# linnil1/KIR_graph

Hardware: AMD Instinct MI355X
Metric: typed 150 bp PE reads/s (pileup+EM) per GPU; achieved HBM GB/s vs roofline (higher is better)
Workload: dtype f64

## Files before the change

include/graphkir_hip.h:

```cpp
#ifndef GRAPHKIR_HIP_H
#define GRAPHKIR_HIP_H

#include <stddef.h>
#include <stdint.h>

#ifdef __cplusplus
extern "C" {
#endif

#define GK_ABI_VERSION 1

#define GK_OK 0
#define GK_ERR_NO_DEVICE (-1)
#define GK_ERR_HIP (-2)
#define GK_ERR_ARG (-3)
#define GK_ERR_ASSERT (-4)
#define GK_ERR_CAPACITY (-5)

#define GK_MAX_CIG 14
#define GK_MAX_MM 16
#define GK_MAX_INS 6
#define GK_MAX_EVENTS 22
#define GK_CIG_M 0
#define GK_CIG_I 1
// ... 23 lines not shown

#define GK_SPILLED 0xFF
#define GK_WIDE_CIG 128
#define GK_WIDE_MM 256
#define GK_WIDE_INS 120
#define GK_WIDE_EVENTS 384
typedef struct gk_mate_wide {
  uint32_t pos0;
  uint16_t flag;
  uint8_t ref;
  uint8_t nh;
  uint8_t nm;
  uint8_t rsv0;
  uint16_t n_cig;
  uint16_t n_mm;
  uint16_t n_ins;
  uint32_t cig[GK_WIDE_CIG];
  uint32_t mm[GK_WIDE_MM];
  uint32_t ins[GK_WIDE_INS];
  uint8_t rsv1[16];
} gk_mate_wide;

typedef struct gk_ctx gk_ctx;
typedef struct gk_index gk_index;
typedef struct gk_tab gk_tab;
typedef struct gk_lut gk_lut;
typedef uint64_t gk_dptr;

int gk_abi_version(void);
const char* gk_last_error(void);
int gk_device_count(int* n);
int gk_ctx_create(int device, gk_ctx** out);
int gk_ctx_create_priority(int device, int urgent, gk_ctx** out);
int gk_ctx_destroy(gk_ctx* ctx);
int gk_sync(gk_ctx* ctx);
int gk_device_memory(gk_ctx* ctx, int64_t* free_bytes, int64_t* total_bytes, int64_t* pool_cached_bytes);
int gk_malloc(gk_ctx* ctx, size_t bytes, gk_dptr* out);
int gk_free(gk_ctx* ctx, gk_dptr p);
int gk_memset(gk_ctx* ctx, gk_dptr p, int value, size_t bytes);
int gk_h2d(gk_ctx* ctx, gk_dptr dst, const void* src, size_t bytes);
int gk_d2h(gk_ctx* ctx, void* dst, gk_dptr src, size_t bytes);
int gk_d2d(gk_ctx* ctx, gk_dptr dst, gk_dptr src, size_t bytes);
int gk_timer_start(gk_ctx* ctx);
int gk_timer_stop_ms(gk_ctx* ctx, float* ms);
int gk_prof_enable(gk_ctx* ctx, int on);
int gk_prof_kernel_count(void);
const char* gk_prof_kernel_name(int id);
int gk_prof_collect(gk_ctx* ctx, int64_t* launches, double* total_ms);

int gk_index_create(gk_ctx* ctx, const uint64_t* key, int32_t n_var, const int32_t* gene_vbeg,
                    int32_t n_gene, gk_index** out);
int gk_index_destroy(gk_index* idx);

typedef struct gk_tab_info {
  int64_t n_pairs;
  int64_t n_valid;
  int64_t n_ids;
  int32_t n_novel;
  int32_t err_flags;
  gk_dptr d_pair_src;
  gk_dptr d_off;
  gk_dptr d_ids;
  gk_dptr d_pair_gene;
  gk_dptr d_pair_nh;
  gk_dptr d_novel_key;
} gk_tab_info;
int gk_tabulate(gk_ctx* ctx, gk_index* idx, gk_dptr d_mates, int64_t n_pairs, gk_tab** out);
int gk_tabulate_corrected(gk_ctx* ctx, gk_index* idx, gk_dptr d_mates, int64_t n_pairs, gk_dptr d_corr,
                          gk_dptr d_gene_pos0, gk_tab** out);
int gk_tabulate_spilled(gk_ctx* ctx, gk_index* idx, gk_dptr d_mates, int64_t n_pairs, gk_dptr d_corr,
                        gk_dptr d_gene_pos0, const gk_mate_wide* wide, const int64_t* spill_pair, int64_t n_spill,
                        gk_tab** out);
#define GK_COMPACT_STAGE_WORDS 4352
int gk_tabulate_compact(gk_ctx* ctx, gk_index* idx, gk_dptr d_compact, int64_t n_pairs, gk_dptr d_corr,
                        gk_dptr d_gene_pos0, const gk_mate_wide* wide, const int64_t* spill_pair, int64_t n_spill,
                        gk_tab** out);
int gk_tab_from_csr(gk_ctx* ctx, int32_t n_var_total, int64_t n_valid, const uint32_t* off, const uint32_t* ids,
                    const uint8_t* pair_gene, const uint8_t* pair_nh, gk_tab** out);
int gk_tab_get_info(gk_tab* tab, gk_tab_info* info);
int gk_tab_destroy(gk_tab* tab);

int gk_select_gene(gk_ctx* ctx, gk_tab* tab, int gene, int multiple, gk_dptr d_rows_out, int64_t* n_out);
int gk_select_nonempty(gk_ctx* ctx, gk_tab* tab, gk_dptr d_rows, int64_t n_rows, gk_dptr d_vflag,
                       gk_dptr d_rows_out, int64_t* n_out);

int gk_variant_count(gk_ctx* ctx, gk_tab* tab, gk_dptr d_rows, int64_t n_rows, gk_dptr d_vflag,
                     gk_dptr d_cnt);
int gk_variant_count_range(gk_ctx* ctx, gk_tab* tab, gk_dptr d_rows, int64_t n_rows, gk_dptr d_vflag,
                           gk_dptr d_cnt, int32_t vbeg, int32_t vend);
int gk_variant_correct(gk_ctx* ctx, gk_tab* tab, gk_dptr d_cnt, gk_dptr d_vflag);
int gk_variant_surviving(gk_ctx* ctx, gk_tab* tab, gk_dptr d_cnt, gk_dptr d_vflag, int64_t max_out,
                         int32_t* ord_out, uint32_t* pos_out, uint32_t* neg_out, int64_t* n_out);

int gk_variant_surviving_gene(gk_ctx* ctx, gk_tab* tab, gk_dptr d_cnt, gk_dptr d_vflag, int32_t gene, int32_t vbeg,
                              int32_t vend, int64_t max_out, int32_t* ord_out, uint32_t* pos_out, uint32_t* neg_out,
                              int64_t* n_out);
int gk_sample_prepare(gk_ctx* ctx, gk_tab* tab, int32_t multiple, gk_dptr d_vflag, gk_dptr d_cnt, gk_dptr d_rows,
                      int64_t* gene_off_out);
int gk_sample_prepare_all(gk_ctx* ctx, gk_tab* tab, int32_t multiple, gk_dptr d_vflag, gk_dptr d_cnt, gk_dptr d_rows,
                          int64_t* gene_off_out, int64_t max_out, int32_t* ord_out, uint32_t* pos_out, uint32_t* neg_out,
                          int64_t* n_out, uint64_t* novel_key_out);
int gk_sample_prepare_exon(gk_ctx* ctx, gk_tab* tab, int32_t multiple, gk_dptr d_vflag, gk_dptr d_cnt, gk_dptr d_rows,
                           int64_t* gene_off_out, int64_t max_out, int32_t* ord_out, uint32_t* pos_out, uint32_t* neg_out,
                           int64_t* n_out);
int gk_sample_prepare_exon_from(gk_ctx* ctx, gk_tab* tab, int32_t multiple, gk_dptr d_vflag, gk_dptr d_cnt, gk_dptr d_rows,
                                int64_t* gene_off_out, int64_t max_out, int32_t* ord_out, uint32_t* pos_out,
                                uint32_t* neg_out, int64_t* n_out, gk_dptr d_cnt_full);

int gk_compat(gk_ctx* ctx, gk_tab* tab, gk_dptr d_rows, int64_t n_rows, gk_dptr d_vflag,
              int32_t vbeg, int32_t vend, gk_dptr d_mask, int32_t words, int32_t n_allele, int32_t keep_empty,
              gk_dptr d_probs, gk_dptr d_miss, gk_dptr d_nvar);

int gk_novel_assign(gk_ctx* ctx, gk_dptr d_probs, int64_t n_rows, int32_t n_cols, const uint32_t* col_entries,
                    int32_t n_entries, gk_dptr d_code, uint16_t* code_out, uint32_t* count_out, int32_t* first_out);
int gk_novel_confusion(gk_ctx* ctx, gk_tab* tab, gk_dptr d_rows, int64_t n_rows, gk_dptr d_code, gk_dptr d_vflag,
                       int32_t vbeg, int32_t vend, gk_dptr d_carry, const int32_t* entry_col, const int32_t* entry_slot,
                       int32_t n_entries, int32_t n_slots, uint64_t* totals_out, int64_t max_out, int32_t* slot_out,
                       int32_t* ord_out, uint32_t* count_out, uint64_t* key_out, int64_t* n_out);

int gk_lut_create(gk_ctx* ctx, int32_t log2_capacity, gk_lut** out);
int gk_lut_destroy(gk_lut* lut);
int gk_lut_collect(gk_lut* lut, gk_dptr d_vals, int64_t n);
int gk_lut_pending(gk_lut* lut, int32_t* n_total, int32_t* n_known);
int gk_lut_export(gk_lut* lut, int32_t first, int32_t count, double* keys_out);
int gk_lut_define(gk_lut* lut, int32_t first, int32_t count, const double* log_vals);
int gk_lut_apply(gk_lut* lut, gk_dptr d_in, gk_dptr d_out, int64_t n);
typedef int (*gk_log10_fn)(const double* values, int64_t n, double* out);
int gk_lut_resolve(gk_lut* lut, gk_log10_fn log10_fn, int32_t* n_new, int32_t* n_known, int32_t* n_undefined);
int gk_lut_resolve_stored(gk_lut* lut, gk_log10_fn log10_fn, int32_t* n_new, int32_t* n_known, int32_t* n_undefined);
int gk_lut_known(gk_lut* lut, int32_t* n_known);
int gk_compat_log(gk_ctx* ctx, gk_tab* tab, gk_dptr d_rows, int64_t n_rows, gk_dptr d_vflag,
                  int32_t vbeg, int32_t vend, gk_dptr d_mask, int32_t words, int32_t n_allele, int32_t keep_empty,
                  gk_lut* lut, gk_dptr d_log);

int gk_maxsum(gk_ctx* ctx, gk_dptr d_L, int64_t n_rows, int64_t ld, const int32_t* ids, int32_t n_sets,
              int32_t c_prev, const int32_t* cols, int32_t n_cols, double* out);
int gk_fraction(gk_ctx* ctx, gk_dptr d_L, int64_t n_rows, int64_t ld, const int32_t* ids,
                int32_t n_sets, int32_t c, double* frac_out);
int gk_setmax(gk_ctx* ctx, gk_dptr d_L, int64_t n_rows, int64_t ld, const int32_t* ids, int32_t n_sets,
              int32_t c, gk_dptr d_P);

int gk_compat_log_miss(gk_ctx* ctx, gk_tab* tab, gk_dptr d_rows, int64_t n_rows, gk_dptr d_vflag,
                       int32_t vbeg, int32_t vend, gk_dptr d_mask, int32_t words, int32_t n_allele,
                       int32_t keep_empty, gk_lut* lut, gk_dptr d_log, gk_dptr d_miss8, int64_t ldm, gk_dptr d_flags);
int gk_miss_colsum(gk_ctx* ctx, gk_dptr d_miss8, int64_t ldm, int32_t n_cols, gk_dptr d_msum);
int gk_compat_log_miss_cols(gk_ctx* ctx, gk_tab* tab, gk_dptr d_rows, int64_t n_rows, gk_dptr d_vflag,
                            int32_t vbeg, int32_t vend, gk_dptr d_mask, int32_t words, int32_t n_allele,
                            int32_t keep_empty, gk_lut* lut, const int32_t* table_cols, int32_t n_table_cols,
                            gk_dptr d_log, gk_dptr d_miss8, int64_t ldm, gk_dptr d_flags);
int gk_compat_log_miss_narrow(gk_ctx* ctx, gk_tab* tab, gk_dptr d_rows, int64_t n_rows, gk_dptr d_vflag,
                              int32_t vbeg, int32_t vend, gk_dptr d_mask, int32_t words, int32_t n_allele,
                              int32_t keep_empty, gk_lut* lut, const int32_t* table_cols, int32_t n_table_cols,
                              gk_dptr d_log, gk_dptr d_miss8, int64_t ldm, gk_dptr d_flags, gk_dptr d_msum);
int gk_compat_patch(gk_ctx* ctx, gk_lut* lut, gk_dptr d_log, int64_t n_rows, int32_t n_allele, gk_dptr d_miss8,
                    int64_t ldm, gk_dptr d_flags);
int gk_compat_index(gk_ctx* ctx, gk_tab* tab, gk_dptr d_rows, int64_t n_rows, gk_dptr d_vflag, int32_t vbeg,
                    int32_t vend, gk_dptr d_mask, int32_t words, int32_t n_allele, int32_t keep_empty, gk_lut* lut,
                    gk_dptr d_lidx, gk_dptr d_miss8, int64_t ldm, gk_dptr d_flags);
int gk_expand_index(gk_ctx* ctx, gk_lut* lut, gk_dptr d_lidx, int64_t ldi, int64_t n_rows, int32_t n_allele, gk_dptr d_L,
                    int64_t ld);
int gk_bound_step(gk_ctx* ctx, gk_dptr d_miss8, int64_t ldm, int64_t n_rows, gk_dptr d_msum, const int32_t* ids,
                  int32_t n_sets, int32_t c_prev, const int32_t* cols, int32_t n_cols, const uint8_t* first,
                  int32_t top_n, int32_t cap, uint32_t* hdr_out, int32_t* idx_out, uint32_t* m_out);
int gk_setsum(gk_ctx* ctx, gk_dptr d_L, int64_t n_rows, int64_t ld, const int32_t* ids, int32_t n_sets, int32_t c,
              double* value_out, double* frac_out);

typedef int (*gk_argsort_fn)(const double* values, int64_t n, int64_t* order_out);
typedef struct gk_search gk_search;
int gk_search_run(gk_ctx* ctx, gk_dptr d_L, int64_t n_rows, int64_t ld, int32_t n_allele, gk_dptr d_miss8,
                  int64_t ldm, gk_dptr d_msum, const int32_t* cols, int32_t n_cols, int32_t n_steps, int32_t top_n,
                  gk_argsort_fn argsort, const double* colsum_in, gk_search** out);
typedef struct gk_gene_job {
  gk_dptr d_rows;
  int64_t n_rows;
  gk_dptr d_mask;
  gk_dptr d_L;
  gk_dptr d_miss8;
  int64_t ldm;
  gk_dptr d_msum;
  gk_dptr d_flags;
  gk_dptr d_lidx;
  int32_t vbeg, vend;
  int32_t words, n_allele;
  int32_t n_steps, top_n;
  int32_t bound_ok, passes;
  int32_t indexed, patches;
  int32_t table_of, n_step_cols;
  const int32_t* step_cols;
  const int32_t* step_cols_off;
  const int32_t* table_cols;
  int32_t n_table_cols;
} gk_gene_job;
int gk_sample_search(gk_ctx* ctx, gk_ctx** more_ctx, int32_t n_more, gk_tab* tab, gk_dptr d_vflag, gk_lut* lut,
                     gk_gene_job* jobs, int32_t n_jobs, gk_argsort_fn argsort, gk_log10_fn log10_fn, gk_search** out);
int gk_search_steps(gk_search* s, int32_t* n_steps);
int gk_search_info(gk_search* s, int32_t step, int32_t* n, int64_t* rows, int32_t* bounded);
int gk_search_copy(gk_search* s, int32_t step, double* value, double* sum_indv, int32_t* ids, double* frac);
int gk_search_export(gk_search* const* s, int32_t n, int64_t* totals, int64_t* meta, double* value, double* sum_indv,
                     double* frac, int32_t* ids);
int gk_search_colsum(gk_search* s, double* out);
int gk_search_log(gk_search* s, int64_t* out, int64_t capacity, int64_t* n_out);
int gk_search_destroy(gk_search* s);
int gk_site_verdict(const int64_t* pos, const int64_t* code, const uint8_t* negative, const int64_t* count, int64_t n,
                    int32_t cn, int32_t* homozygous);
int gk_site_verdict_tallies(const uint64_t* keys, int64_t n_keys, const int64_t* label_of_insert, int64_t n_insert,
                            const int32_t* ordinal, const uint32_t* positive, const uint32_t* negative, int64_t n,
                            int32_t cn, int32_t* homozygous);
int gk_site_verdict_genes(const uint64_t* keys, int64_t n_keys, const int64_t* label_of_insert, int64_t n_insert,
                          const int32_t* ordinal, const uint32_t* positive, const uint32_t* negative,
                          const int64_t* bounds, int32_t n_groups, const int32_t* cn, int32_t* homozygous);

int gk_em_sets(gk_ctx* ctx, gk_tab* tab, gk_dptr d_rows, int64_t n_rows, int32_t vbeg, int32_t vend,
               gk_dptr d_mask, int32_t words, gk_dptr d_sets_out );
int gk_em_distinct(gk_ctx* ctx, gk_dptr d_sets, int64_t n_rows, int32_t words, int32_t max_out,
                   uint32_t* sets_out, uint32_t* count_out, int32_t* n_out);
int gk_em_run(gk_ctx* ctx, const uint32_t* sets, const double* weight, int32_t n_sets, int32_t words,
              int32_t n_allele, int32_t iter_max, double diff_threshold, double* prob_out,
              int32_t* iters_out);
typedef struct gk_em_job {
  gk_dptr d_rows;
  int64_t n_rows;
  gk_dptr d_mask;
  int32_t vbeg, vend;
  int32_t words, n_allele;
  int32_t n_distinct, iterations;
} gk_em_job;
int gk_sample_em(gk_ctx* ctx, gk_tab* tab, gk_em_job* jobs, int32_t n_jobs, int32_t iter_max, double diff_threshold,
                 double* prob_out, int64_t* count_out);

typedef struct gk_boot_job {
  const uint32_t* sets;
  const uint32_t* count;
  int32_t n_sets;
  int32_t words;
  int32_t n_allele;
  uint32_t stream;
} gk_boot_job;
int gk_em_bootstrap(gk_ctx* ctx, const gk_boot_job* jobs, int32_t n_jobs, int32_t n_boot, uint64_t seed,
                    int32_t iter_max, double diff_threshold,
                    double* prob_out,
                    int32_t* iters_out,
                    uint32_t* counts_out);

int gk_boot_row_counts(gk_ctx* ctx, int64_t n_rows, int32_t n_boot, int32_t boot_first, uint64_t seed, uint32_t stream,
                       gk_dptr d_W, int64_t ldw);
int gk_weighted_sums(gk_ctx* ctx, gk_dptr d_V, int64_t ld, int64_t n_rows, int32_t n_sets, gk_dptr d_W, int64_t ldw,
                     int32_t n_boot, double* out);

int gk_call_fit(gk_ctx* ctx, gk_dptr d_miss8, int64_t ldm, int64_t n_rows, int32_t n_table_cols, const int32_t* cols,
                int32_t n_cols, uint64_t* hist_out , uint64_t* col_out , uint64_t* m_out ,
                gk_dptr d_min);
int gk_call_fit_extra(gk_ctx* ctx, gk_dptr d_miss8, int64_t ldm, int64_t n_rows, int32_t n_table_cols, gk_dptr d_min,
                      uint64_t* with_out );

int gk_call_coverage(gk_ctx* ctx, gk_tab* tab, gk_dptr d_mates, gk_dptr d_compact, gk_dptr d_rows, int64_t n_rows,
                     gk_dptr d_miss8, int64_t ldm, int32_t n_table_cols, const int32_t* cols, int32_t n_cols, int32_t gene,
                     int64_t gene_len, uint32_t* depth_out );

typedef struct gk_packer gk_packer;
int gk_packer_create(const char* const* gene_names, int32_t n_genes, const char* const* ins_strings,
                     int32_t n_ins, gk_packer** out);
int gk_packer_destroy(gk_packer* pk);
int gk_packer_feed(gk_packer* pk, const char* text, size_t n_bytes, int32_t final);
int gk_packer_counts(gk_packer* pk, int64_t* n_lines, int64_t* n_reads, int64_t* n_pairs, int64_t* n_strange,
                     int64_t* n_strings);
int gk_packer_error(gk_packer* pk, int32_t* kind, int64_t* line_index);
int gk_packer_set_output(gk_packer* pk, gk_mate* mates_out, int64_t capacity);
int gk_packer_records(gk_packer* pk, gk_mate* mates_out, int64_t* pair_lines_out);
int gk_packer_spilled(gk_packer* pk, int64_t* n_spilled_pairs);
int gk_packer_spill_records(gk_packer* pk, gk_mate_wide* wide_out, int64_t* pair_index_out);
const char* gk_packer_string(gk_packer* pk, int64_t i);

typedef struct gk_bam gk_bam;
int gk_bam_open(const char* path, int32_t name_sorted, gk_bam** out);
int gk_bam_close(gk_bam* bam);
int gk_bam_info(gk_bam* bam, int64_t* n_records, int64_t* header_bytes, int32_t* n_ref);
int gk_bam_header(gk_bam* bam, char* text_out, int64_t capacity);
int gk_bam_next(gk_bam* bam, char* text_out, int64_t capacity, int64_t* n_written);
int gk_bam_pack(gk_bam* bam, struct gk_packer* packer);
int gk_bam_write(const char* path, const char* sam_text, int64_t n_bytes, int32_t coordinate_sort);
int gk_bam_write_lines(const char* path, const char* header_text, int64_t n_header, const char* sam_text,
                       int64_t n_bytes, const int64_t* line_idx, int64_t n_lines, int32_t coordinate_sort);
int gk_json_write_reads(const char* path, const char* sam_text, int64_t n_bytes, const int64_t* pair_lines,
                        int64_t n_pairs, const int64_t* src, int64_t n_rows, const uint32_t* off,
                        const uint32_t* ids, const char* const* names, int64_t n_names,
                        const char* const* genes, int32_t n_genes, const uint8_t* gene_of, const uint8_t* nh);
int gk_bam_pileup(gk_bam* bam, const int64_t* gene_off, int32_t n_gene, uint32_t* counts_out);
int gk_bam_pileup_sites(const char* path, const int64_t* sites, int64_t n_sites, const uint64_t* name_keys,
                        const int32_t* key_group, int64_t n_keys, const int32_t* site_group, uint32_t* counts_out);
int gk_sam_name_keys(const char* sam_text, int64_t n_bytes, const int64_t* line_idx, int64_t n_lines, uint64_t* keys_out);
int gk_bam_write_lines_tagged(const char* path, const char* header_text, int64_t n_header, const char* rg_text,
                              int64_t n_rg, const char* sam_text, int64_t n_bytes, const int64_t* line_idx,
                              const int32_t* line_group, int64_t n_lines, const char* const* tags, int32_t n_tags,
                              int32_t coordinate_sort);

int gk_depth(gk_ctx* ctx, gk_tab* tab, gk_dptr d_mates, int32_t multiple, const int64_t* gene_off,
             int32_t n_gene, uint32_t* depth_out);
int gk_depth_compact(gk_ctx* ctx, gk_tab* tab, gk_dptr d_compact, int32_t multiple, const int64_t* gene_off,
                     int32_t n_gene, uint32_t* depth_out);

int gk_depth_write_tsv(const char* path, const char* const* genes, const int64_t* gene_off, int32_t n_genes,
                       const uint32_t* depth);

int gk_cn_fit(gk_ctx* ctx, const double* x, const double* density, int32_t bins, const double* bases,
              int32_t n_bases, const double* dev, int32_t n_cn, int32_t first_cn, double space,
              double* loglik_out);
int gk_cn_assign(gk_ctx* ctx, const double* x, int32_t bins, double base, const double* dev, int32_t n_cn,
                 int32_t first_cn, double space, int32_t* cn_of_bin_out);

typedef struct gk_comm gk_comm;
int gk_comm_unique_id(void* id_out, size_t capacity);
int gk_comm_create(gk_ctx* ctx, const void* id, size_t id_bytes, int32_t rank, int32_t world, gk_comm** out);
int gk_comm_destroy(gk_comm* comm);
int gk_allgather_f64(gk_comm* comm, const double* send, double* recv, int64_t n);
int gk_allreduce_max_f64(gk_comm* comm, double* inout, int64_t n);
int gk_comm_barrier(gk_comm* comm);

int gk_mates_compact(gk_ctx* ctx, gk_dptr d_mates, int64_t n_mates, gk_dptr* d_compact_out, int64_t* bytes_out);
int gk_mates_expand(gk_ctx* ctx, gk_dptr d_compact, int64_t n_mates, gk_dptr d_mates_out);
int gk_mates_compact_size(const gk_mate* mates, int64_t n_mates, int32_t n_threads, int64_t* n_words_out);
int gk_mates_compact_host(const gk_mate* mates, int64_t n_mates, int32_t n_threads, uint32_t* out, int64_t capacity_words);

int gk_host_alloc(size_t bytes, void** out);
int gk_host_free(void* p);
int gk_h2d_async(gk_ctx* ctx, gk_dptr dst, const void* src, size_t bytes);

#ifdef __cplusplus
}
#endif
#endif
```

kir_graph_amd/_lib.py:

```python
from __future__ import annotations

import ctypes as C
import threading
import os
from pathlib import Path

import numpy as np

LIB_NAME = "libgraphkir_hip.so"
_lib = None


class GkError(RuntimeError):
    """Error reported by the native library."""


class GkNoDevice(GkError):
    """No HIP device: the typing path cannot run (there is no CPU fallback)."""


_MM = np.dtype([("ref_off", "<u2"), ("base", "u1"), ("rsv", "u1")])
MATE_DTYPE = np.dtype([
    ("pos0", "<u4"), ("flag", "<u2"), ("ref", "u1"), ("nh", "u1"),
    ("nm", "u1"), ("n_cig", "u1"), ("n_mm", "u1"), ("n_ins", "u1"),
    ("cig", "<u2", (14,)), ("mm", _MM, (16,)), ("ins", "<u4", (6,)),
])
assert MATE_DTYPE.itemsize == 128

MATE_WIDE_DTYPE = np.dtype([
    ("pos0", "<u4"), ("flag", "<u2"), ("ref", "u1"), ("nh", "u1"), ("nm", "u1"), ("rsv0", "u1"),
    ("n_cig", "<u2"), ("n_mm", "<u2"), ("n_ins", "<u2"),
    ("cig", "<u4", (128,)), ("mm", "<u4", (256,)), ("ins", "<u4", (120,)), ("rsv1", "u1", (16,)),
])
assert MATE_WIDE_DTYPE.itemsize == 2048
SPILLED = 0xFF

CIG_M, CIG_I, CIG_D, CIG_S = 0, 1, 2, 4
NM_ABSENT = 255
MAX_CIG, MAX_MM, MAX_INS, MAX_EV = 14, 16, 6, 22
COMPACT_STAGE_WORDS = 4352


class GeneJob(C.Structure):
    _fields_ = [
        ("d_rows", C.c_uint64), ("n_rows", C.c_int64), ("d_mask", C.c_uint64), ("d_L", C.c_uint64),
        ("d_miss8", C.c_uint64), ("ldm", C.c_int64), ("d_msum", C.c_uint64), ("d_flags", C.c_uint64),
        ("d_lidx", C.c_uint64),
        ("vbeg", C.c_int32), ("vend", C.c_int32), ("words", C.c_int32), ("n_allele", C.c_int32),
        ("n_steps", C.c_int32), ("top_n", C.c_int32), ("bound_ok", C.c_int32), ("passes", C.c_int32),
        ("indexed", C.c_int32), ("patches", C.c_int32),
        ("table_of", C.c_int32), ("n_step_cols", C.c_int32), ("step_cols", C.c_void_p), ("step_cols_off", C.c_void_p),
        ("table_cols", C.c_void_p), ("n_table_cols", C.c_int32),
    ]


class EmJob(C.Structure):
    _fields_ = [
        ("d_rows", C.c_uint64), ("n_rows", C.c_int64), ("d_mask", C.c_uint64),
        ("vbeg", C.c_int32), ("vend", C.c_int32), ("words", C.c_int32), ("n_allele", C.c_int32),
        ("n_distinct", C.c_int32), ("iterations", C.c_int32),
    ]


class BootJob(C.Structure):
    _fields_ = [
        ("sets", C.c_void_p), ("count", C.c_void_p),
        ("n_sets", C.c_int32), ("words", C.c_int32), ("n_allele", C.c_int32), ("stream", C.c_uint32),
    ]


class TabInfo(C.Structure):
    _fields_ = [
        ("n_pairs", C.c_int64), ("n_valid", C.c_int64), ("n_ids", C.c_int64),
        ("n_novel", C.c_int32), ("err_flags", C.c_int32),
        ("d_pair_src", C.c_uint64), ("d_off", C.c_uint64), ("d_ids", C.c_uint64),
        ("d_pair_gene", C.c_uint64), ("d_pair_nh", C.c_uint64), ("d_novel_key", C.c_uint64),
    ]


def libPath() -> Path:
    return Path(__file__).resolve().parent / LIB_NAME


_SIGS = {
    "gk_abi_version": (C.c_int, []),
    "gk_last_error": (C.c_char_p, []),
    "gk_device_count": (C.c_int, [C.POINTER(C.c_int)]),
    "gk_ctx_create": (C.c_int, [C.c_int, C.POINTER(C.c_void_p)]),
    "gk_ctx_create_priority": (C.c_int, [C.c_int, C.c_int, C.POINTER(C.c_void_p)]),
    "gk_ctx_destroy": (C.c_int, [C.c_void_p]),
    "gk_sync": (C.c_int, [C.c_void_p]),
    "gk_device_memory": (C.c_int, [C.c_void_p, C.POINTER(C.c_int64), C.POINTER(C.c_int64), C.POINTER(C.c_int64)]),
    "gk_malloc": (C.c_int, [C.c_void_p, C.c_size_t, C.POINTER(C.c_uint64)]),
    "gk_free": (C.c_int, [C.c_void_p, C.c_uint64]),
    "gk_memset": (C.c_int, [C.c_void_p, C.c_uint64, C.c_int, C.c_size_t]),
    "gk_h2d": (C.c_int, [C.c_void_p, C.c_uint64, C.c_void_p, C.c_size_t]),
    "gk_d2h": (C.c_int, [C.c_void_p, C.c_void_p, C.c_uint64, C.c_size_t]),
    "gk_d2d": (C.c_int, [C.c_void_p, C.c_uint64, C.c_uint64, C.c_size_t]),
    "gk_timer_start": (C.c_int, [C.c_void_p]),
    "gk_timer_stop_ms": (C.c_int, [C.c_void_p, C.POINTER(C.c_float)]),
    "gk_prof_enable": (C.c_int, [C.c_void_p, C.c_int]),
    "gk_prof_kernel_count": (C.c_int, []),
    "gk_prof_kernel_name": (C.c_char_p, [C.c_int]),
    "gk_prof_collect": (C.c_int, [C.c_void_p, C.c_void_p, C.c_void_p]),
    "gk_index_create": (C.c_int, [C.c_void_p, C.c_void_p, C.c_int32, C.c_void_p, C.c_int32, C.POINTER(C.c_void_p)]),
    "gk_index_destroy": (C.c_int, [C.c_void_p]),
    "gk_tabulate": (C.c_int, [C.c_void_p, C.c_void_p, C.c_uint64, C.c_int64, C.POINTER(C.c_void_p)]),
    "gk_tabulate_spilled": (C.c_int, [C.c_void_p, C.c_void_p, C.c_uint64, C.c_int64, C.c_uint64, C.c_uint64,
                                     C.c_void_p, C.c_void_p, C.c_int64, C.POINTER(C.c_void_p)]),
    "gk_tabulate_corrected": (C.c_int, [C.c_void_p, C.c_void_p, C.c_uint64, C.c_int64, C.c_uint64, C.c_uint64,
                                        C.POINTER(C.c_void_p)]),
    "gk_tabulate_compact": (C.c_int, [C.c_void_p, C.c_void_p, C.c_uint64, C.c_int64, C.c_uint64, C.c_uint64,
                                     C.c_void_p, C.c_void_p, C.c_int64, C.POINTER(C.c_void_p)]),
    "gk_tab_from_csr": (C.c_int, [C.c_void_p, C.c_int32, C.c_int64, C.c_void_p, C.c_void_p, C.c_void_p, C.c_void_p,
                                  C.POINTER(C.c_void_p)]),
    "gk_tab_get_info": (C.c_int, [C.c_void_p, C.POINTER(TabInfo)]),
    "gk_tab_destroy": (C.c_int, [C.c_void_p]),
    "gk_select_gene": (C.c_int, [C.c_void_p, C.c_void_p, C.c_int, C.c_int, C.c_uint64, C.POINTER(C.c_int64)]),
    "gk_select_nonempty": (C.c_int, [C.c_void_p, C.c_void_p, C.c_uint64, C.c_int64, C.c_uint64, C.c_uint64,
                                     C.POINTER(C.c_int64)]),
    "gk_variant_count": (C.c_int, [C.c_void_p, C.c_void_p, C.c_uint64, C.c_int64, C.c_uint64, C.c_uint64]),
    "gk_variant_count_range": (C.c_int, [C.c_void_p, C.c_void_p, C.c_uint64, C.c_int64, C.c_uint64, C.c_uint64,
                                         C.c_int32, C.c_int32]),
    "gk_variant_surviving": (C.c_int, [C.c_void_p, C.c_void_p, C.c_uint64, C.c_uint64, C.c_int64, C.c_void_p,
                                       C.c_void_p, C.c_void_p, C.POINTER(C.c_int64)]),
    "gk_variant_surviving_gene": (C.c_int, [C.c_void_p, C.c_void_p, C.c_uint64, C.c_uint64, C.c_int32, C.c_int32, C.c_int32,
                                            C.c_int64, C.c_void_p, C.c_void_p, C.c_void_p, C.POINTER(C.c_int64)]),
    "gk_sample_prepare": (C.c_int, [C.c_void_p, C.c_void_p, C.c_int32, C.c_uint64, C.c_uint64, C.c_uint64, C.c_void_p]),
    "gk_sample_prepare_all": (C.c_int, [C.c_void_p, C.c_void_p, C.c_int32, C.c_uint64, C.c_uint64, C.c_uint64, C.c_void_p,
                                       C.c_int64, C.c_void_p, C.c_void_p, C.c_void_p, C.POINTER(C.c_int64), C.c_void_p]),
    "gk_variant_correct": (C.c_int, [C.c_void_p, C.c_void_p, C.c_uint64, C.c_uint64]),
    "gk_compat": (C.c_int, [C.c_void_p, C.c_void_p, C.c_uint64, C.c_int64, C.c_uint64, C.c_int32, C.c_int32,
                            C.c_uint64, C.c_int32, C.c_int32, C.c_int32, C.c_uint64, C.c_uint64, C.c_uint64]),
    "gk_lut_create": (C.c_int, [C.c_void_p, C.c_int32, C.POINTER(C.c_void_p)]),
    "gk_lut_destroy": (C.c_int, [C.c_void_p]),
    "gk_lut_collect": (C.c_int, [C.c_void_p, C.c_uint64, C.c_int64]),
    "gk_lut_pending": (C.c_int, [C.c_void_p, C.POINTER(C.c_int32), C.POINTER(C.c_int32)]),
    "gk_lut_export": (C.c_int, [C.c_void_p, C.c_int32, C.c_int32, C.c_void_p]),
    "gk_lut_define": (C.c_int, [C.c_void_p, C.c_int32, C.c_int32, C.c_void_p]),
    "gk_lut_apply": (C.c_int, [C.c_void_p, C.c_uint64, C.c_uint64, C.c_int64]),
    "gk_bam_open": (C.c_int, [C.c_char_p, C.c_int32, C.POINTER(C.c_void_p)]),
    "gk_bam_close": (C.c_int, [C.c_void_p]),
    "gk_bam_info": (C.c_int, [C.c_void_p, C.POINTER(C.c_int64), C.POINTER(C.c_int64), C.POINTER(C.c_int32)]),
    "gk_bam_header": (C.c_int, [C.c_void_p, C.c_char_p, C.c_int64]),
    "gk_bam_pileup": (C.c_int, [C.c_void_p, C.c_void_p, C.c_int32, C.c_void_p]),
    "gk_bam_pileup_sites": (C.c_int, [C.c_char_p, C.c_void_p, C.c_int64, C.c_void_p, C.c_void_p, C.c_int64, C.c_void_p,
                                      C.c_void_p]),
    "gk_sam_name_keys": (C.c_int, [C.c_char_p, C.c_int64, C.c_void_p, C.c_int64, C.c_void_p]),
    "gk_bam_write_lines_tagged": (C.c_int, [C.c_char_p, C.c_char_p, C.c_int64, C.c_char_p, C.c_int64, C.c_char_p,
                                            C.c_int64, C.c_void_p, C.c_void_p, C.c_int64, C.c_void_p, C.c_int32,
                                            C.c_int32]),
    "gk_novel_assign": (C.c_int, [C.c_void_p, C.c_uint64, C.c_int64, C.c_int32, C.c_void_p, C.c_int32, C.c_uint64,
                                  C.c_void_p, C.c_void_p, C.c_void_p]),
    "gk_novel_confusion": (C.c_int, [C.c_void_p, C.c_void_p, C.c_uint64, C.c_int64, C.c_uint64, C.c_uint64, C.c_int32,
                                     C.c_int32, C.c_uint64, C.c_void_p, C.c_void_p, C.c_int32, C.c_int32, C.c_void_p,
                                     C.c_int64, C.c_void_p, C.c_void_p, C.c_void_p, C.c_void_p, C.POINTER(C.c_int64)]),
    "gk_bam_write": (C.c_int, [C.c_char_p, C.c_char_p, C.c_int64, C.c_int32]),
    "gk_bam_write_lines": (C.c_int, [C.c_char_p, C.c_char_p, C.c_int64, C.c_char_p, C.c_int64, C.c_void_p, C.c_int64,
                                     C.c_int32]),
    "gk_json_write_reads": (C.c_int, [C.c_char_p, C.c_char_p, C.c_int64, C.c_void_p, C.c_int64, C.c_void_p, C.c_int64,
                                      C.c_void_p, C.c_void_p, C.c_void_p, C.c_int64, C.c_void_p, C.c_int32,
                                      C.c_void_p, C.c_void_p]),
    "gk_bam_pack": (C.c_int, [C.c_void_p, C.c_void_p]),
    "gk_bam_next": (C.c_int, [C.c_void_p, C.c_void_p, C.c_int64, C.POINTER(C.c_int64)]),
    "gk_compat_log": (C.c_int, [C.c_void_p, C.c_void_p, C.c_uint64, C.c_int64, C.c_uint64, C.c_int32, C.c_int32,
                                C.c_uint64, C.c_int32, C.c_int32, C.c_int32, C.c_void_p, C.c_uint64]),
    "gk_maxsum": (C.c_int, [C.c_void_p, C.c_uint64, C.c_int64, C.c_int64, C.c_void_p, C.c_int32, C.c_int32,
                            C.c_void_p, C.c_int32, C.c_void_p]),
    "gk_fraction": (C.c_int, [C.c_void_p, C.c_uint64, C.c_int64, C.c_int64, C.c_void_p, C.c_int32, C.c_int32,
                              C.c_void_p]),
    "gk_setmax": (C.c_int, [C.c_void_p, C.c_uint64, C.c_int64, C.c_int64, C.c_void_p, C.c_int32, C.c_int32,
                            C.c_uint64]),
    "gk_packer_create": (C.c_int, [C.c_void_p, C.c_int32, C.c_void_p, C.c_int32, C.POINTER(C.c_void_p)]),
    "gk_packer_destroy": (C.c_int, [C.c_void_p]),
    "gk_packer_feed": (C.c_int, [C.c_void_p, C.c_char_p, C.c_size_t, C.c_int32]),
    "gk_packer_counts": (C.c_int, [C.c_void_p, C.POINTER(C.c_int64), C.POINTER(C.c_int64), C.POINTER(C.c_int64),
                                   C.POINTER(C.c_int64), C.POINTER(C.c_int64)]),
    "gk_packer_error": (C.c_int, [C.c_void_p, C.POINTER(C.c_int32), C.POINTER(C.c_int64)]),
    "gk_packer_records": (C.c_int, [C.c_void_p, C.c_void_p, C.c_void_p]),
    "gk_packer_set_output": (C.c_int, [C.c_void_p, C.c_void_p, C.c_int64]),
    "gk_packer_spilled": (C.c_int, [C.c_void_p, C.POINTER(C.c_int64)]),
    "gk_packer_spill_records": (C.c_int, [C.c_void_p, C.c_void_p, C.c_void_p]),
    "gk_packer_string": (C.c_char_p, [C.c_void_p, C.c_int64]),
    "gk_depth": (C.c_int, [C.c_void_p, C.c_void_p, C.c_uint64, C.c_int32, C.c_void_p, C.c_int32, C.c_void_p]),
    "gk_depth_compact": (C.c_int, [C.c_void_p, C.c_void_p, C.c_uint64, C.c_int32, C.c_void_p, C.c_int32, C.c_void_p]),
    "gk_depth_write_tsv": (C.c_int, [C.c_char_p, C.c_void_p, C.c_void_p, C.c_int32, C.c_void_p]),
    "gk_cn_fit": (C.c_int, [C.c_void_p, C.c_void_p, C.c_void_p, C.c_int32, C.c_void_p, C.c_int32, C.c_void_p,
                            C.c_int32, C.c_int32, C.c_double, C.c_void_p]),
    "gk_cn_assign": (C.c_int, [C.c_void_p, C.c_void_p, C.c_int32, C.c_double, C.c_void_p, C.c_int32, C.c_int32,
                               C.c_double, C.c_void_p]),
    "gk_em_sets": (C.c_int, [C.c_void_p, C.c_void_p, C.c_uint64, C.c_int64, C.c_int32, C.c_int32, C.c_uint64,
                             C.c_int32, C.c_uint64]),
    "gk_em_distinct": (C.c_int, [C.c_void_p, C.c_uint64, C.c_int64, C.c_int32, C.c_int32, C.c_void_p, C.c_void_p,
                                 C.POINTER(C.c_int32)]),
    "gk_compat_log_miss_cols": (C.c_int, [C.c_void_p, C.c_void_p, C.c_uint64, C.c_int64, C.c_uint64, C.c_int32, C.c_int32,
                                          C.c_uint64, C.c_int32, C.c_int32, C.c_int32, C.c_void_p, C.c_void_p, C.c_int32,
                                          C.c_uint64, C.c_uint64, C.c_int64, C.c_uint64]),
    "gk_compat_log_miss_narrow": (C.c_int, [C.c_void_p, C.c_void_p, C.c_uint64, C.c_int64, C.c_uint64, C.c_int32, C.c_int32,
                                            C.c_uint64, C.c_int32, C.c_int32, C.c_int32, C.c_void_p, C.c_void_p, C.c_int32,
                                            C.c_uint64, C.c_uint64, C.c_int64, C.c_uint64, C.c_uint64]),
    "gk_compat_log_miss": (C.c_int, [C.c_void_p, C.c_void_p, C.c_uint64, C.c_int64, C.c_uint64, C.c_int32, C.c_int32,
                                     C.c_uint64, C.c_int32, C.c_int32, C.c_int32, C.c_void_p, C.c_uint64, C.c_uint64,
                                     C.c_int64, C.c_uint64]),
    "gk_miss_colsum": (C.c_int, [C.c_void_p, C.c_uint64, C.c_int64, C.c_int32, C.c_uint64]),
    "gk_compat_index": (C.c_int, [C.c_void_p, C.c_void_p, C.c_uint64, C.c_int64, C.c_uint64, C.c_int32, C.c_int32,
                                  C.c_uint64, C.c_int32, C.c_int32, C.c_int32, C.c_void_p, C.c_uint64, C.c_uint64,
                                  C.c_int64, C.c_uint64]),
    "gk_expand_index": (C.c_int, [C.c_void_p, C.c_void_p, C.c_uint64, C.c_int64, C.c_int64, C.c_int32, C.c_uint64,
                                  C.c_int64]),
    "gk_bound_step": (C.c_int, [C.c_void_p, C.c_uint64, C.c_int64, C.c_int64, C.c_uint64, C.c_void_p, C.c_int32,
                                C.c_int32, C.c_void_p, C.c_int32, C.c_void_p, C.c_int32, C.c_int32, C.c_void_p,
                                C.c_void_p, C.c_void_p]),
    "gk_setsum": (C.c_int, [C.c_void_p, C.c_uint64, C.c_int64, C.c_int64, C.c_void_p, C.c_int32, C.c_int32,
                            C.c_void_p, C.c_void_p]),
    "gk_search_run": (C.c_int, [C.c_void_p, C.c_uint64, C.c_int64, C.c_int64, C.c_int32, C.c_uint64, C.c_int64,
                                C.c_uint64, C.c_void_p, C.c_int32, C.c_int32, C.c_int32, C.c_void_p, C.c_void_p,
                                C.POINTER(C.c_void_p)]),
    "gk_sample_search": (C.c_int, [C.c_void_p, C.c_void_p, C.c_int32, C.c_void_p, C.c_uint64, C.c_void_p, C.c_void_p,
                                   C.c_int32, C.c_void_p, C.c_void_p, C.c_void_p]),
    "gk_lut_resolve": (C.c_int, [C.c_void_p, C.c_void_p, C.POINTER(C.c_int32), C.POINTER(C.c_int32),
                                 C.POINTER(C.c_int32)]),
    "gk_sample_prepare_exon": (C.c_int, [C.c_void_p, C.c_void_p, C.c_int32, C.c_uint64, C.c_uint64, C.c_uint64, C.c_void_p,
                                         C.c_int64, C.c_void_p, C.c_void_p, C.c_void_p, C.POINTER(C.c_int64)]),
    "gk_sample_prepare_exon_from": (C.c_int, [C.c_void_p, C.c_void_p, C.c_int32, C.c_uint64, C.c_uint64, C.c_uint64, C.c_void_p,
                                              C.c_int64, C.c_void_p, C.c_void_p, C.c_void_p, C.POINTER(C.c_int64), C.c_uint64]),
    "gk_sample_em": (C.c_int, [C.c_void_p, C.c_void_p, C.c_void_p, C.c_int32, C.c_int32, C.c_double, C.c_void_p, C.c_void_p]),
    "gk_mates_compact": (C.c_int, [C.c_void_p, C.c_uint64, C.c_int64, C.POINTER(C.c_uint64), C.POINTER(C.c_int64)]),
    "gk_mates_expand": (C.c_int, [C.c_void_p, C.c_uint64, C.c_int64, C.c_uint64]),
    "gk_mates_compact_size": (C.c_int, [C.c_void_p, C.c_int64, C.c_int32, C.POINTER(C.c_int64)]),
    "gk_mates_compact_host": (C.c_int, [C.c_void_p, C.c_int64, C.c_int32, C.c_void_p, C.c_int64]),
    "gk_compat_patch": (C.c_int, [C.c_void_p, C.c_void_p, C.c_uint64, C.c_int64, C.c_int32, C.c_uint64, C.c_int64, C.c_uint64]),
    "gk_lut_resolve_stored": (C.c_int, [C.c_void_p, C.c_void_p, C.POINTER(C.c_int32), C.POINTER(C.c_int32),
                                        C.POINTER(C.c_int32)]),
    "gk_lut_known": (C.c_int, [C.c_void_p, C.POINTER(C.c_int32)]),
    "gk_search_steps": (C.c_int, [C.c_void_p, C.POINTER(C.c_int32)]),
    "gk_search_info": (C.c_int, [C.c_void_p, C.c_int32, C.POINTER(C.c_int32), C.POINTER(C.c_int64),
                                 C.POINTER(C.c_int32)]),
    "gk_search_copy": (C.c_int, [C.c_void_p, C.c_int32, C.c_void_p, C.c_void_p, C.c_void_p, C.c_void_p]),
    "gk_search_export": (C.c_int, [C.c_void_p, C.c_int32, C.c_void_p, C.c_void_p, C.c_void_p, C.c_void_p, C.c_void_p, C.c_void_p]),
    "gk_search_colsum": (C.c_int, [C.c_void_p, C.c_void_p]),
    "gk_search_log": (C.c_int, [C.c_void_p, C.c_void_p, C.c_int64, C.POINTER(C.c_int64)]),
    "gk_search_destroy": (C.c_int, [C.c_void_p]),
    "gk_site_verdict_tallies": (C.c_int, [C.c_void_p, C.c_int64, C.c_void_p, C.c_int64, C.c_void_p, C.c_void_p, C.c_void_p,
                                         C.c_int64, C.c_int32, C.POINTER(C.c_int32)]),
    "gk_site_verdict_genes": (C.c_int, [C.c_void_p, C.c_int64, C.c_void_p, C.c_int64, C.c_void_p, C.c_void_p, C.c_void_p,
                                       C.c_void_p, C.c_int32, C.c_void_p, C.c_void_p]),
    "gk_site_verdict": (C.c_int, [C.c_void_p, C.c_void_p, C.c_void_p, C.c_void_p, C.c_int64, C.c_int32,
                                  C.POINTER(C.c_int32)]),
    "gk_comm_unique_id": (C.c_int, [C.c_void_p, C.c_size_t]),
    "gk_comm_create": (C.c_int, [C.c_void_p, C.c_void_p, C.c_size_t, C.c_int32, C.c_int32, C.POINTER(C.c_void_p)]),
    "gk_comm_destroy": (C.c_int, [C.c_void_p]),
    "gk_allgather_f64": (C.c_int, [C.c_void_p, C.c_void_p, C.c_void_p, C.c_int64]),
    "gk_allreduce_max_f64": (C.c_int, [C.c_void_p, C.c_void_p, C.c_int64]),
    "gk_comm_barrier": (C.c_int, [C.c_void_p]),
    "gk_host_alloc": (C.c_int, [C.c_size_t, C.POINTER(C.c_void_p)]),
    "gk_host_free": (C.c_int, [C.c_void_p]),
    "gk_h2d_async": (C.c_int, [C.c_void_p, C.c_uint64, C.c_void_p, C.c_size_t]),
    "gk_em_run": (C.c_int, [C.c_void_p, C.c_void_p, C.c_void_p, C.c_int32, C.c_int32, C.c_int32, C.c_int32,
                            C.c_double, C.c_void_p, C.POINTER(C.c_int32)]),
    "gk_em_bootstrap": (C.c_int, [C.c_void_p, C.c_void_p, C.c_int32, C.c_int32, C.c_uint64, C.c_int32, C.c_double,
                                  C.c_void_p, C.c_void_p, C.c_void_p]),
    "gk_boot_row_counts": (C.c_int, [C.c_void_p, C.c_int64, C.c_int32, C.c_int32, C.c_uint64, C.c_uint32, C.c_uint64,
                                     C.c_int64]),
    "gk_weighted_sums": (C.c_int, [C.c_void_p, C.c_uint64, C.c_int64, C.c_int64, C.c_int32, C.c_uint64, C.c_int64, C.c_int32,
                                   C.c_void_p]),
    "gk_call_fit": (C.c_int, [C.c_void_p, C.c_uint64, C.c_int64, C.c_int64, C.c_int32, C.c_void_p, C.c_int32, C.c_void_p,
                              C.c_void_p, C.c_void_p, C.c_uint64]),
    "gk_call_fit_extra": (C.c_int, [C.c_void_p, C.c_uint64, C.c_int64, C.c_int64, C.c_int32, C.c_uint64, C.c_void_p]),
    "gk_call_coverage": (C.c_int, [C.c_void_p, C.c_void_p, C.c_uint64, C.c_uint64, C.c_uint64, C.c_int64, C.c_uint64, C.c_int64,
                                   C.c_int32, C.c_void_p, C.c_int32, C.c_int32, C.c_int64, C.c_void_p]),
}

EXPORTED = sorted(_SIGS)

ARGSORT_FN = C.CFUNCTYPE(C.c_int, C.POINTER(C.c_double), C.c_int64, C.POINTER(C.c_int64))


def _numpy_argsort(values, n, order_out):
    try:
        v = np.ctypeslib.as_array(values, shape=(n,))
        np.ctypeslib.as_array(order_out, shape=(n,))[:] = np.argsort(v)
        return 0
    except Exception:
        return 1


NUMPY_ARGSORT = ARGSORT_FN(_numpy_argsort)

LOG10_FN = C.CFUNCTYPE(C.c_int, C.POINTER(C.c_double), C.c_int64, C.POINTER(C.c_double))


def _numpy_log10(values, n, out):
    try:
        v = np.ctypeslib.as_array(values, shape=(n,))
        with np.errstate(divide="ignore"):
            np.ctypeslib.as_array(out, shape=(n,))[:] = np.log10(v)
        return 0
    except Exception:
        return 1


NUMPY_LOG10 = LOG10_FN(_numpy_log10)


def lib():
    global _lib
    if _lib is None:
        path = libPath()
        if not path.exists():
            raise GkError(
                f"{path} is missing: build it with `python -c 'import __graft_entry__ as g; g.build()'` "
                "(hipcc --offload-arch=gfx950). The typing path has no CPU fallback.")
        handle = C.CDLL(str(path))
        for name, (res, args) in _SIGS.items():
            fn = getattr(handle, name)
            fn.restype, fn.argtypes = res, args
        if handle.gk_abi_version() != 1:
            raise GkError("libgraphkir_hip.so ABI version mismatch")
        _lib = handle
    return _lib


def check(rc: int) -> None:
    if rc == 0:
        return
    msg = lib().gk_last_error().decode(errors="replace")
    if rc == -1:
        raise GkNoDevice(msg)
    if rc == -4:
        raise AssertionError(msg)
    raise GkError(f"[{rc}] {msg}")


def _np_ptr(a: np.ndarray) -> C.c_void_p:
    return C.c_void_p(a.ctypes.data)


class DeviceBuffer:

    def __init__(self, dev: "Device", shape, dtype):
        self.dev = dev
        self.shape = tuple(int(s) for s in (shape if isinstance(shape, (tuple, list)) else (shape,)))
        self.dtype = np.dtype(dtype)
        self.nbytes = int(np.prod(self.shape, dtype=np.int64)) * self.dtype.itemsize
        p = C.c_uint64()
        check(lib().gk_malloc(dev.ctx, max(self.nbytes, 16), C.byref(p)))
        self.ptr = p.value

    @property
    def size(self) -> int:
        return int(np.prod(self.shape, dtype=np.int64))

    def upload(self, a: np.ndarray) -> "DeviceBuffer":
        a = np.ascontiguousarray(a, dtype=self.dtype)
        assert a.nbytes == self.nbytes, (a.shape, self.shape)
        if a.nbytes:
            check(lib().gk_h2d(self.dev.ctx, self.ptr, _np_ptr(a), a.nbytes))
# ... 175 lines not shown
```

kir_graph_amd/build.py:

```python
from __future__ import annotations

import os
import shutil
import subprocess
from pathlib import Path

PKG = Path(__file__).resolve().parent
ROOT = PKG.parent
SOURCES = ["gk_runtime.hip", "gk_scan.hip", "gk_tabulate.hip", "gk_typing.hip", "gk_lut.hip",
           "gk_search.hip", "gk_bound.hip", "gk_em.hip", "gk_cn.hip", "gk_depth.hip", "gk_sampack.cpp", "gk_bamread.cpp", "gk_textout.cpp",
           "gk_comm.cpp", "gk_hostsearch.cpp", "gk_novel.hip", "gk_boot.hip", "gk_callboot.hip", "gk_compat_narrow.hip",
           "gk_callfit.hip", "gk_callcov.hip"]


def hipcc() -> str:
    for cand in (os.environ.get("HIPCC"), shutil.which("hipcc"), "/opt/rocm/bin/hipcc"):
        if cand and Path(cand).exists():
            return cand
    raise RuntimeError("hipcc not found (set HIPCC)")


def outOfDate(lib: Path) -> bool:
    if not lib.exists():
        return True
    t = lib.stat().st_mtime
    deps = [PKG / "csrc" / s for s in SOURCES] + list((PKG / "csrc").glob("*.h")) + [ROOT / "include" / "graphkir_hip.h"]
    return any(d.stat().st_mtime > t for d in deps)


KERNEL_SOURCES = {
    "compat_kernel": ["gk_typing.hip", "gk_lut.h", "gk_common.h"],
    "patch_pending": ["gk_typing.hip", "gk_lut.h", "gk_common.h"],
    "compat_rows8": ["gk_compat_narrow.hip", "gk_lut.h", "gk_common.h"],
    "count_ids_genes": ["gk_typing.hip", "gk_common.h"],
    "flag_nonempty": ["gk_typing.hip", "gk_common.h"],
    "flag_pairs": ["gk_typing.hip", "gk_common.h"],
    "gather_pair_flags": ["gk_typing.hip", "gk_common.h"],
    "tab_count": ["gk_tabulate.hip", "gk_common.h"],
    "tab_emit": ["gk_tabulate.hip", "gk_common.h"],
    "tab_expand": ["gk_tabulate.hip", "gk_common.h"],
    "minsum_sad": ["gk_bound.hip", "gk_common.h"],
    "minsum_finish": ["gk_bound.hip", "gk_common.h"],
    "select_hist1": ["gk_bound.hip", "gk_common.h"],
    "select_hist2": ["gk_bound.hip", "gk_common.h"],
    "select_append": ["gk_bound.hip", "gk_common.h"],
    "setmin_u8": ["gk_bound.hip", "gk_common.h"],
    "fraction_chunks": ["gk_search.hip", "gk_common.h"],
    "setsum_leaves": ["gk_search.hip", "gk_common.h"],
    "fold_leaves": ["gk_search.hip", "gk_common.h"],
    "colsum_chunks": ["gk_search.hip", "gk_common.h"],
    "maxsum_chunks": ["gk_search.hip", "gk_common.h"],
    "combine_chunks": ["gk_search.hip", "gk_common.h"],
    "em_sets_groups": ["gk_em.hip", "gk_common.h"],
    "em_sets_hash": ["gk_em.hip", "gk_common.h"],
    "em_sets_verify": ["gk_em.hip", "gk_common.h"],
    "em_sets_emit": ["gk_em.hip", "gk_common.h"],
    "em_kernel_genes": ["gk_em.hip", "gk_squarem.h", "gk_common.h"],
    "novel_assign": ["gk_novel.hip", "gk_common.h"],
    "novel_confusion": ["gk_novel.hip", "gk_common.h"],
    "novel_compact": ["gk_novel.hip", "gk_common.h"],
    "boot_resample": ["gk_boot.hip", "gk_common.h"],
    "boot_em_batch": ["gk_boot.hip", "gk_squarem.h", "gk_common.h"],
    "callboot_draw": ["gk_callboot.hip", "gk_common.h"],
    "callboot_sums": ["gk_callboot.hip", "gk_common.h"],
    "callboot_fold": ["gk_callboot.hip", "gk_common.h"],
    "callfit_profile": ["gk_callfit.hip", "gk_common.h"],
    "callfit_extra": ["gk_callfit.hip", "gk_common.h"],
    "callcov_mark": ["gk_callcov.hip", "gk_common.h"],
    "callcov_mark_lds": ["gk_callcov.hip", "gk_common.h"],
    "callcov_finish": ["gk_callcov.hip", "gk_common.h"],
}


def sourceDigest(kernel: str | None = None) -> str:
    import hashlib
    h = hashlib.sha256()
    names = KERNEL_SOURCES.get(kernel or "")
    if names is None:
        files = sorted((PKG / "csrc").glob("*.hip")) + sorted((PKG / "csrc").glob("*.h"))
    else:
        files = [PKG / "csrc" / n for n in names]
    for f in files:
        h.update(f.name.encode())
        h.update(f.read_bytes())
    return h.hexdigest()[:16]


EXTRA_FLAGS: dict[str, list[str]] = {}


def buildNative(force: bool = False, verbose: bool = False) -> Path:
    lib = PKG / "libgraphkir_hip.so"
    if not force and not outOfDate(lib):
        return lib
    objdir = PKG / "csrc" / "build"
    objdir.mkdir(exist_ok=True)
    base = [hipcc(), "-O3", "--offload-arch=gfx950", "-std=c++17", "-fPIC", "-Wno-unused-value",
            "-Wno-unused-result", f"-I{ROOT / 'include'}", f"-I{PKG / 'csrc'}"]
    jobs = []
    for src in SOURCES:
        obj = objdir / (src.rsplit(".", 1)[0] + ".o")
        cmd = base + EXTRA_FLAGS.get(src, []) + ["-c", str(PKG / "csrc" / src), "-o", str(obj)]
        if verbose:
            print(" ".join(cmd))
        jobs.append((src, obj, subprocess.Popen(cmd, stdout=subprocess.PIPE, stderr=subprocess.PIPE, text=True)))
    failed = []
    for src, obj, proc in jobs:
        out, err = proc.communicate()
        if proc.returncode != 0:
            failed.append(f"{src}:\n{out}\n{err}")
    if failed:
        raise RuntimeError("hipcc failed:\n" + "\n".join(failed))
    link = [hipcc(), "--offload-arch=gfx950", "-shared", "-fPIC", "-o", str(lib)] + [str(o) for _, o, _ in jobs] + ["-lz", "-ldl"]
    if verbose:
        print(" ".join(link))
    res = subprocess.run(link, capture_output=True, text=True)
    if res.returncode != 0:
        raise RuntimeError(f"link failed:\n{res.stdout}\n{res.stderr}")
    return lib


if __name__ == "__main__":
    print(buildNative(force=True, verbose=True))
```

kir_graph_amd/csrc/gk_hostsearch.cpp:

```cpp
#include <algorithm>
#include <cmath>
#include <memory>
#include <numeric>
#include <string>
#include <unordered_map>
#include <unordered_set>
#include <chrono>
#include <sys/syscall.h>
#include <unistd.h>

#include "gk_calls.h"
#include "gk_lut.h"

namespace {

struct Step {
  int n = 0;
  int bounded = 0;
  std::vector<double> value, sum_indv, frac;
  std::vector<int32_t> ids;
  int64_t rows() const { return (int64_t)value.size(); }
};

inline double sum_small(const double* a, int n) {
// ... 24 lines not shown
    for (int a = 0; a < A && unique_cols; ++a) {
      if (seen[cols[a]]) unique_cols = false;
      seen[cols[a]] = 1;
    }
  }
  if (k <= 2 && n_allele <= 2048 && unique_cols) {
    std::vector<char> offered((size_t)n_allele, 0);
    for (int a = 0; a < A; ++a) offered[cols[a]] = 1;
    if (k == 1) {
      std::vector<int32_t> pos((size_t)n_allele, T);
      for (int t = T - 1; t >= 0; --t) pos[prev[t]] = t;
      for (int t = 0; t < T; ++t) {
        const int p = prev[t];
        if (pos[p] != t) continue;
        const bool free_pass = !offered[p];
        uint8_t* row = first.data() + (size_t)t * A;
        for (int a = 0; a < A; ++a) row[a] = (free_pass || pos[cols[a]] >= t) ? 1 : 0;
      }
      return;
    }
    std::vector<int32_t> pos((size_t)n_allele * n_allele, T);
    for (int t = T - 1; t >= 0; --t) {
      const int lo = std::min(prev[2 * t], prev[2 * t + 1]), hi = std::max(prev[2 * t], prev[2 * t + 1]);
      pos[(size_t)lo * n_allele + hi] = t;
      pos[(size_t)hi * n_allele + lo] = t;
    }
    for (int t = 0; t < T; ++t) {
      const int lo = std::min(prev[2 * t], prev[2 * t + 1]), hi = std::max(prev[2 * t], prev[2 * t + 1]);
      if (pos[(size_t)lo * n_allele + hi] != t) continue;
      const int32_t* by_hi = pos.data() + (size_t)hi * n_allele;
      const int32_t* by_lo = pos.data() + (size_t)lo * n_allele;
      const bool lo_off = offered[lo], hi_off = offered[hi];
      uint8_t* row = first.data() + (size_t)t * A;
      for (int a = 0; a < A; ++a) {
        const int c = cols[a];
        const bool dup = (by_hi[c] < t && lo_off) || (by_lo[c] < t && hi_off);
        row[a] = dup ? 0 : 1;
      }
    }
    return;
  }
  std::unordered_set<std::string> seen;
  seen.reserve((size_t)T * A * 2);
  std::vector<int32_t> key((size_t)k + 1);
  for (int t = 0; t < T; ++t)
    for (int a = 0; a < A; ++a) {
      std::copy(prev + (size_t)t * k, prev + (size_t)(t + 1) * k, key.begin());
      key[k] = cols[a];
      std::sort(key.begin(), key.end());
      std::string s((const char*)key.data(), key.size() * sizeof(int32_t));
      first[(size_t)t * A + a] = seen.insert(std::move(s)).second ? 1 : 0;
    }
}

struct Head {
  int c = 0;
  std::vector<int32_t> ids;
  std::vector<double> value;
  std::vector<double> sum_indv;
  std::vector<double> key2;
};

void fill_sums(Head& h, const double* colsum) {
  const int64_t n = (int64_t)h.value.size();
  h.sum_indv.resize((size_t)n * h.c);
  h.key2.resize((size_t)n);
  for (int64_t i = 0; i < n; ++i) {
    double* s = h.sum_indv.data() + (size_t)i * h.c;
    for (int j = 0; j < h.c; ++j) s[j] = colsum[h.ids[(size_t)i * h.c + j]];
    h.key2[i] = -sum_small(s, h.c);
  }
}

void contenders(const Head& h, int top_n, std::vector<int64_t>& contend) {
  const int64_t n = (int64_t)h.value.size();
  contend.clear();
  if (n <= top_n) {
    contend.resize((size_t)n);
    std::iota(contend.begin(), contend.end(), 0);
    return;
  }
  std::vector<int64_t> order((size_t)n);
  std::iota(order.begin(), order.end(), 0);
  std::stable_sort(order.begin(), order.end(), [&](int64_t a, int64_t b) {
    const double ka = -h.value[a], kb = -h.value[b];
    if (ka != kb) return ka < kb;
    return h.key2[a] < h.key2[b];
  });
  const int64_t b = order[top_n - 1];
  const double b1 = -h.value[b], b2 = h.key2[b];
  for (int64_t i = 0; i < n; ++i) {
    const double k1 = -h.value[i];
    if (k1 < b1 || (k1 == b1 && h.key2[i] <= b2)) contend.push_back(i);
  }
}

double unevenness(const double* f, int c) {
  const double mean = sum_small(f, c) / (double)c;
  double d[8];
  for (int j = 0; j < c; ++j) d[j] = std::fabs(f[j] - mean);
  return sum_small(d, c);
}

}

struct gk_search {
  int n_allele = 0;
  std::vector<int32_t> table_cols;
  int n_full = 0;
  std::vector<double> colsum;
  std::vector<Step> steps;
  std::vector<int64_t> log;
  int64_t distinct(const int32_t* ids, size_t n) const {
    std::vector<char> seen((size_t)n_allele, 0);
    int64_t d = 0;
    for (size_t i = 0; i < n; ++i)
      if (!seen[ids[i]]) { seen[ids[i]] = 1; ++d; }
    return d;
  }
  void note(int64_t kind, int64_t a, int64_t b, int64_t c, int64_t d, int64_t e, int64_t f) {
    const int64_t row[7] = {kind, a, b, c, d, e, f};
    log.insert(log.end(), row, row + 7);
  }
  void to_alleles(const int32_t* cols, int n_cols, int n_alleles) {
    for (Step& st : steps)
      for (int32_t& id : st.ids) id = cols[id];
    table_cols.assign(cols, cols + n_cols);
    n_full = n_alleles;
  }
};

extern "C" {

int gk_maxsum(gk_ctx* ctx, gk_dptr d_L, int64_t n_rows, int64_t ld, const int32_t* ids, int32_t n_sets, int32_t c_prev,
              const int32_t* cols, int32_t n_cols, double* out);
int gk_fraction(gk_ctx* ctx, gk_dptr d_L, int64_t n_rows, int64_t ld, const int32_t* ids, int32_t n_sets, int32_t c,
                double* frac_out);
int gk_compat_log_miss(gk_ctx* ctx, gk_tab* tab, gk_dptr d_rows, int64_t n_rows, gk_dptr d_vflag, int32_t vbeg,
                       int32_t vend, gk_dptr d_mask, int32_t words, int32_t n_allele, int32_t keep_empty, gk_lut* lut,
                       gk_dptr d_log, gk_dptr d_miss8, int64_t ldm, gk_dptr d_flags);
int gk_compat_log(gk_ctx* ctx, gk_tab* tab, gk_dptr d_rows, int64_t n_rows, gk_dptr d_vflag, int32_t vbeg,
                  int32_t vend, gk_dptr d_mask, int32_t words, int32_t n_allele, int32_t keep_empty, gk_lut* lut,
                  gk_dptr d_log);
__attribute__((weak)) int gk_compat_log_miss_cols(gk_ctx* ctx, gk_tab* tab, gk_dptr d_rows, int64_t n_rows, gk_dptr d_vflag,
                                                  int32_t vbeg, int32_t vend, gk_dptr d_mask, int32_t words, int32_t n_allele,
                                                  int32_t keep_empty, gk_lut* lut, const int32_t* table_cols,
                                                  int32_t n_table_cols, gk_dptr d_log, gk_dptr d_miss8, int64_t ldm,
                                                  gk_dptr d_flags);
__attribute__((weak)) int gk_compat_log_miss_narrow(gk_ctx* ctx, gk_tab* tab, gk_dptr d_rows, int64_t n_rows, gk_dptr d_vflag,
                                                    int32_t vbeg, int32_t vend, gk_dptr d_mask, int32_t words, int32_t n_allele,
                                                    int32_t keep_empty, gk_lut* lut, const int32_t* table_cols,
                                                    int32_t n_table_cols, gk_dptr d_log, gk_dptr d_miss8, int64_t ldm,
                                                    gk_dptr d_flags, gk_dptr d_msum);
int gk_miss_colsum(gk_ctx* ctx, gk_dptr d_miss8, int64_t ldm, int32_t n_cols, gk_dptr d_msum);
int gk_compat_patch(gk_ctx* ctx, gk_lut* lut, gk_dptr d_log, int64_t n_rows, int32_t n_allele, gk_dptr d_miss8, int64_t ldm,
                    gk_dptr d_flags);
int gk_compat_index(gk_ctx* ctx, gk_tab* tab, gk_dptr d_rows, int64_t n_rows, gk_dptr d_vflag, int32_t vbeg, int32_t vend,
                    gk_dptr d_mask, int32_t words, int32_t n_allele, int32_t keep_empty, gk_lut* lut, gk_dptr d_lidx,
                    gk_dptr d_miss8, int64_t ldm, gk_dptr d_flags);

}

namespace {

struct GeneSearch {
  gk_ctx* ctx = nullptr;
  GkTable table;
  gk_dptr d_L = 0;
  void* expanded = nullptr;
  gk_dptr d_miss8 = 0, d_msum = 0;
  int64_t n_rows = 0, ld = 0, ldm = 0;
  int n_allele = 0, n_steps = 0, T = 0, A = 0;
  std::vector<int32_t> cols;
  std::vector<std::vector<int32_t>> step_cols;
  gk_argsort_fn argsort = nullptr;
  bool bound = false, unique_cols = true;
  std::unique_ptr<gk_search> S;
  std::vector<uint8_t> first;
  int64_t N = 0;
  GkBoundCall bcall;
  GkSumCall scall;
  Head sel;
  Step st;
  bool bound_in_flight = false, sums_in_flight = false, step_done = false;

  int init(gk_ctx* c, const GkTable& tbl, gk_dptr L, int64_t rows, int64_t ld_, int32_t n_allele_, gk_dptr miss8, int64_t ldm_,
           gk_dptr msum, const int32_t* cols_, int32_t n_cols, int32_t n_steps_, int32_t top_n, gk_argsort_fn fn) {
    GK_REQUIRE(c && tbl.d && (L || tbl.indexed()) && cols_ && fn, "null pointer");
    table = tbl;
    GK_REQUIRE(rows > 0 && ld_ >= rows && n_allele_ > 0 && n_cols > 0 && n_steps_ >= 0 && n_steps_ <= 8 && top_n >= 1,
               "bad search arguments");
    for (int a = 0; a < n_cols; ++a) GK_REQUIRE(cols_[a] >= 0 && cols_[a] < n_allele_, "candidate allele out of range");
    ctx = c; d_L = L; n_rows = rows; ld = ld_; n_allele = n_allele_; d_miss8 = miss8; ldm = ldm_; d_msum = msum;
    cols.assign(cols_, cols_ + n_cols);
    n_steps = n_steps_; T = top_n; A = n_cols; argsort = fn;
    bound = d_miss8 != 0 && d_msum != 0;
    S.reset(new gk_search());
    S->n_allele = n_allele;
    S->colsum.resize((size_t)n_allele);
    std::vector<char> seen((size_t)n_allele, 0);
    for (int a = 0; a < A && unique_cols; ++a) { if (seen[cols[a]]) unique_cols = false; seen[cols[a]] = 1; }
    return GK_OK;
  }

  int use_step(int s) {
    if (step_cols.empty()) return GK_OK;
    const std::vector<int32_t>& c = step_cols[std::min<size_t>((size_t)s, step_cols.size() - 1)];
    GK_REQUIRE(!c.empty(), "a search step without candidate alleles");
    cols = c;
    A = (int)cols.size();
    unique_cols = true;
    std::vector<char> seen((size_t)n_allele, 0);
    for (int a = 0; a < A; ++a) {
      GK_REQUIRE(cols[a] >= 0 && cols[a] < n_allele, "candidate allele out of range");
      if (seen[cols[a]]) unique_cols = false;
      seen[cols[a]] = 1;
    }
    return GK_OK;
  }

  int colsum_enqueue() {
    std::vector<int32_t> every((size_t)n_allele);
    std::iota(every.begin(), every.end(), 0);
    int rc = gk_colsum_enqueue(ctx, table, n_rows, every.data(), n_allele, scall);
    if (rc) return rc;
    S->note(0, n_rows, 1, 0, n_allele, 0, 0);
    return GK_OK;
  }
  void colsum_collect() { gk_colsum_collect(ctx, scall, S->colsum.data()); }

  int first_step() {
    { const int r = use_step(0); if (r) return r; }
    const double* colsum = S->colsum.data();
    std::vector<double> score((size_t)A);
    for (int a = 0; a < A; ++a) score[a] = colsum[cols[a]];
    std::vector<int64_t> order((size_t)A);
    bool plain = true;
    for (int a = 0; a < A && plain; ++a) plain = score[a] == score[a];
    if (plain) {
      std::iota(order.begin(), order.end(), 0);
      std::sort(order.begin(), order.end(), [&](int64_t x, int64_t y) { return score[x] != score[y] ? score[x] < score[y] : x < y; });
      for (int a = 1; a < A && plain; ++a) plain = score[order[a - 1]] != score[order[a]];
    }
    if (!plain) GK_REQUIRE(argsort(score.data(), A, order.data()) == 0, "host argsort failed");
    Step s1;
    s1.n = 1;
    const int keep = std::min(T, A);
    for (int i = 0; i < keep; ++i) {
      const int64_t a = order[(size_t)A - 1 - i];
      GK_REQUIRE(a >= 0 && a < A, "host argsort returned an index out of range");
      s1.value.push_back(score[a]);
      s1.sum_indv.push_back(score[a]);
      s1.ids.push_back(cols[a]);
      s1.frac.push_back(1.0);
    }
    S->steps.push_back(std::move(s1));
    return GK_OK;
  }

  bool more() const { return (int)S->steps.size() < n_steps; }

  int step_begin() {
    { const int r = use_step((int)S->steps.size()); if (r) return r; }
    const Step& prev = S->steps.back();
    const int k = prev.n;
    const int Tp = (int)prev.rows();
    first_of_sets(prev.ids.data(), Tp, k, cols.data(), A, n_allele, first);
    N = 0;
    for (uint8_t f : first) N += f;
    st = Step();
    st.n = k + 1;
    step_done = bound_in_flight = sums_in_flight = false;
    if (bound && N > 0 && unique_cols) {
      const int cap = 4 * T + 4096;
      int rc = gk_bound_enqueue(ctx, d_miss8, ldm, n_rows, d_msum, prev.ids.data(), Tp, k, cols.data(), A, first.data(), T,
                                cap, bcall);
      if (rc) return rc;
      S->note(1, n_rows, Tp, A, k == 1 ? S->distinct(prev.ids.data(), prev.ids.size()) : Tp, 0, 0);
      bound_in_flight = true;
    }
    return GK_OK;
  }

  int after_bound() {
    if (!bound_in_flight) return GK_OK;
    bound_in_flight = false;
    const Step& prev = S->steps.back();
    const int k = prev.n, c = k + 1;
    const int cap = bcall.cap;
    uint32_t hdr[4];
    std::vector<int32_t> idx((size_t)cap);
    std::vector<uint32_t> mm((size_t)cap);
    gk_bound_collect(ctx, bcall, hdr, idx.data(), mm.data());
    const int64_t n_sel = hdr[2];
    if (n_sel <= 0 || n_sel > cap) return GK_OK;
    idx.resize((size_t)n_sel);
    std::sort(idx.begin(), idx.end());
    sel = Head();
    sel.c = c;
    sel.ids.resize((size_t)n_sel * c);
    for (int64_t i = 0; i < n_sel; ++i) {
      const int t = idx[i] / A, a = idx[i] % A;
      std::copy(prev.ids.begin() + (size_t)t * k, prev.ids.begin() + (size_t)(t + 1) * k, sel.ids.begin() + (size_t)i * c);
      sel.ids[(size_t)i * c + k] = cols[a];
    }
    int rc = gk_shares_enqueue(ctx, table, n_rows, sel.ids.data(), (int32_t)n_sel, c, true, scall);
// ... 270 lines not shown
  SearchClock clock("lock-step", (int)live.size());
  auto lap = [&](bool waited) { clock.lap(waited); };
  std::vector<uint32_t> flags((size_t)n_jobs, 0);
  std::vector<std::unique_ptr<GeneSearch>> gs((size_t)n_jobs);
  std::vector<char> sums_queued((size_t)n_jobs, 0);
  auto start_search = [&](int i, gk_dptr d_L, bool indexed) {
    gk_gene_job& j = jobs[i];
    std::vector<int32_t> cols((size_t)j.n_allele);
    std::iota(cols.begin(), cols.end(), 0);
    if (gs[i]) gs[i]->abandon();
    gs[i].reset(new GeneSearch());
    const GkTable tbl = indexed ? GkTable{j.d_lidx, j.ldm, lut->d_vals} : GkTable{d_L, j.n_rows, nullptr};
    int r = gs[i]->init(ctx_of[i], tbl, indexed ? 0 : d_L, j.n_rows, j.n_rows, j.n_allele, j.d_miss8, j.ldm, j.d_msum,
                        cols.data(), j.n_allele, j.n_steps, j.top_n, argsort);
    if (r == GK_OK) r = gs[i]->colsum_enqueue();
    sums_queued[i] = r == GK_OK;
    return r;
  };
  auto quit = [&](int code) {
    for (gk_ctx* c : cx) gk_fetch_cancel(c);
    for (auto& g : gs) if (g) g->abandon();
    return code;
  };
  std::vector<int> dirty(live);
  std::vector<uint32_t> sticky((size_t)n_jobs, 0);
  bool settled = false;
  for (int pass = 0; pass < 64 && !settled; ++pass) {
    int32_t known_at_launch = 0;
    rc = gk_lut_known(lut, &known_at_launch);
    if (rc) return quit(rc);
    for (int i : dirty) {
      gk_gene_job& j = jobs[i];
      gk_ctx* const gc = ctx_of[i];
      if (pass > 0 && j.d_L && j.d_miss8 && j.d_flags && (flags[i] & 12u) == 4u) {
        j.patches++;
        sticky[i] |= flags[i] & 1u;
        rc = gk_compat_patch(gc, lut, j.d_L, j.n_rows, j.n_allele, j.d_miss8, j.ldm, j.d_flags);
        if (rc == GK_OK) rc = gk_miss_colsum(gc, j.d_miss8, j.ldm, j.n_allele, j.d_msum);
        if (rc == GK_OK && gk_fetch_queue(gc, &flags[i], gk_ptr<void>(j.d_flags), sizeof(uint32_t)) != hipSuccess) rc = GK_ERR_HIP;
        if (rc == GK_OK) rc = start_search(i, j.d_L, false);
        if (rc) return quit(rc);
        continue;
      }
      j.passes++;
      sticky[i] = 0;
      if (j.d_lidx && !j.d_L) {
        rc = gk_compat_index(gc, tab, j.d_rows, j.n_rows, d_vflag, j.vbeg, j.vend, j.d_mask, j.words, j.n_allele, 0, lut,
                             j.d_lidx, j.d_miss8, j.ldm, j.d_flags);
        if (rc == GK_OK) rc = gk_miss_colsum(gc, j.d_miss8, j.ldm, j.n_allele, j.d_msum);
        if (rc == GK_OK && gk_fetch_queue(gc, &flags[i], gk_ptr<void>(j.d_flags), sizeof(uint32_t)) != hipSuccess) rc = GK_ERR_HIP;
      } else if (j.d_miss8) {
        rc = gk_compat_log_miss(gc, tab, j.d_rows, j.n_rows, d_vflag, j.vbeg, j.vend, j.d_mask, j.words, j.n_allele, 0, lut,
                                j.d_L, j.d_miss8, j.ldm, j.d_flags);
        if (rc == GK_OK) rc = gk_miss_colsum(gc, j.d_miss8, j.ldm, j.n_allele, j.d_msum);
        if (rc == GK_OK && gk_fetch_queue(gc, &flags[i], gk_ptr<void>(j.d_flags), sizeof(uint32_t)) != hipSuccess) rc = GK_ERR_HIP;
        if (rc == GK_OK) rc = start_search(i, j.d_L, false);
      } else {
        rc = gk_compat_log(gc, tab, j.d_rows, j.n_rows, d_vflag, j.vbeg, j.vend, j.d_mask, j.words, j.n_allele, 0, lut, j.d_L);
        if (rc == GK_OK) rc = start_search(i, j.d_L, false);
      }
      if (rc) return quit(rc);
    }
    lap(false); rc = wait_all(); lap(true);
    if (rc) return quit(rc);
    int32_t n_new = 0, n_known = 0, n_undefined = 0;
    rc = gk_lut_resolve(lut, log10_fn, &n_new, &n_known, &n_undefined);
    if (rc) return quit(rc);
    std::vector<int> again;
    bool unflagged = false;
    for (int i : dirty) {
      if (jobs[i].d_flags) { if (flags[i] & 4u) again.push_back(i); }
      else unflagged = true;
    }
    if (unflagged && (n_known > known_at_launch || n_undefined != 0))
      for (int i : dirty) if (!jobs[i].d_flags) again.push_back(i);
    std::sort(again.begin(), again.end());
    settled = again.empty();
    dirty.swap(again);
  }
  if (!settled) {
    gk_set_error("log10 value table did not settle");
    return quit(GK_ERR_ASSERT);
  }
  std::vector<void*> own_L((size_t)n_jobs, nullptr);
  auto fail = [&](int code) {
    for (gk_ctx* c : cx) gk_fetch_cancel(c);
    for (auto& g : gs) if (g) g->abandon();
    for (int i = 0; i < n_jobs; ++i) gk_pool_free(ctx_of[i], own_L[i]);
    return code;
  };
  for (int i : live) {
    gk_gene_job& j = jobs[i];
    j.indexed = (j.d_lidx && !j.d_L && !(flags[i] & 2u)) ? 1 : 0;
    if (j.d_lidx && !j.d_L && !j.indexed) {
      gk_ctx* const gc = ctx_of[i];
      if (gk_pool_malloc(gc, &own_L[i], (size_t)j.n_allele * (size_t)j.n_rows * sizeof(double)) != hipSuccess) {
        gk_set_error("out of device memory for the float64 table of a gene");
        return fail(GK_ERR_HIP);
      }
      rc = gk_compat_log_miss(gc, tab, j.d_rows, j.n_rows, d_vflag, j.vbeg, j.vend, j.d_mask, j.words, j.n_allele, 0, lut,
                              gk_addr(own_L[i]), j.d_miss8, j.ldm, j.d_flags);
      if (rc == GK_OK) rc = gk_miss_colsum(gc, j.d_miss8, j.ldm, j.n_allele, j.d_msum);
      if (rc == GK_OK && gk_fetch_queue(gc, &flags[i], gk_ptr<void>(j.d_flags), sizeof(uint32_t)) != hipSuccess) rc = GK_ERR_HIP;
      if (rc == GK_OK) rc = wait_stream(gc);
      if (rc) return fail(rc);
      j.passes++;
    }
  }
  bool late = false;
  for (int i : live) {
    gk_gene_job& j = jobs[i];
    j.bound_ok = (j.d_miss8 && ((flags[i] | sticky[i]) & 1u) == 0) ? 1 : 0;
    if (!sums_queued[i]) {
      rc = start_search(i, own_L[i] ? gk_addr(own_L[i]) : j.d_L, j.indexed != 0);
      if (rc) return fail(rc);
      late = true;
    }
    if (!j.bound_ok) gs[i]->bound = false;
  }
  if (late) {
    lap(false); rc = wait_all(); lap(true);
    if (rc) return fail(rc);
  }
  for (int i : live) {
    gs[i]->colsum_collect();
    rc = gs[i]->first_step();
    if (rc) return fail(rc);
  }
  for (;;) {
    std::vector<int> todo;
    for (int i : live) if (gs[i]->more()) todo.push_back(i);
    if (todo.empty()) break;
    for (int i : todo) { rc = gs[i]->step_begin(); if (rc) return fail(rc); }
    lap(false); rc = wait_all(); lap(true);
    if (rc) return fail(rc);
    for (int i : todo) { rc = gs[i]->after_bound(); if (rc) return fail(rc); }
    lap(false); rc = wait_all(); lap(true);
    if (rc) return fail(rc);
    for (int i : todo) { rc = gs[i]->after_sums(); if (rc) return fail(rc); }
    for (int i : todo) {
      if (!gs[i]->step_done) { rc = gs[i]->exact_step(); if (rc) return fail(rc); }
      gs[i]->step_end();
    }
  }
  for (int i : live) {
    gs[i]->finish();
    out[i] = gs[i]->S.release();
  }
  for (int i = 0; i < n_jobs; ++i) gk_pool_free(ctx_of[i], own_L[i]);
  lap(false);
  return GK_OK;
}

int sample_search_pipelined(gk_ctx* ctx, gk_tab* tab, gk_dptr d_vflag, gk_lut* lut, gk_gene_job* jobs, int32_t n_jobs,
                            const std::vector<int>& live, gk_argsort_fn argsort, gk_log10_fn log10_fn, gk_search** out) {
  SearchClock clock("pipelined", (int)live.size());
  std::vector<uint32_t> flags((size_t)n_jobs, 0);
  std::vector<std::unique_ptr<GeneSearch>> gs((size_t)n_jobs);
  enum { kTable, kBound, kSums, kOneSet };
  struct Item { int gene, stage; uint64_t mark; };
  std::deque<Item> queue;
  struct OneSetBatch { GkSumCall call; std::vector<int> deps; int k = 0; std::vector<int32_t> ids; };
  std::vector<std::unique_ptr<OneSetBatch>> batches;
  auto fail = [&](int code) {
    gk_fetch_cancel(ctx);
    for (auto& g : gs) if (g) g->abandon();
    for (auto& b : batches) if (b) gk_release(ctx, b->call.temps);
    return code;
  };
  auto push = [&](int gene, int stage) {
    uint64_t m = 0;
    const int r = set_mark(ctx, &m);
    if (r == GK_OK) queue.push_back({gene, stage, m});
    return r;
  };
  std::vector<uint32_t> sticky((size_t)n_jobs, 0);
  auto n_cols_of = [&](int i) { return jobs[i].n_table_cols > 0 ? jobs[i].n_table_cols : jobs[i].n_allele; };
  auto col_of = [&](int owner, int32_t a, int32_t* col) -> int {
    const gk_gene_job& o = jobs[owner];
    if (a < 0 || a >= o.n_allele) { gk_set_error("candidate allele out of range"); return GK_ERR_ARG; }
    if (o.n_table_cols <= 0) { *col = a; return GK_OK; }
    const int32_t* const end = o.table_cols + o.n_table_cols;
    const int32_t* const at = std::lower_bound(o.table_cols, end, a);
    if (at == end || *at != a) {
      gk_set_error("candidate allele %d is not among the columns of its table", (int)a);
      return GK_ERR_ARG;
    }
    *col = (int32_t)(at - o.table_cols);
    return GK_OK;
  };
  auto write_table = [&](int i, bool patch) -> int {
    gk_gene_job& j = jobs[i];
    const int nc = n_cols_of(i);
    int rc;
    bool summed = false;
    if (patch) {
      j.patches++;
      sticky[i] |= flags[i] & 1u;
      rc = gk_compat_patch(ctx, lut, j.d_L, j.n_rows, nc, j.d_miss8, j.ldm, j.d_flags);
    } else {
      j.passes++;
      sticky[i] = 0;
      static const bool wide_compat = gk_test_hook("wide_compat");
      if (j.n_table_cols > 0 && j.n_table_cols <= 8 && gk_compat_log_miss_narrow && !wide_compat) {
        rc = gk_compat_log_miss_narrow(ctx, tab, j.d_rows, j.n_rows, d_vflag, j.vbeg, j.vend, j.d_mask, j.words, j.n_allele, 0,
                                       lut, j.table_cols, j.n_table_cols, j.d_L, j.d_miss8, j.ldm, j.d_flags, j.d_msum);
        summed = true;
      } else if (j.n_table_cols > 0)
        rc = gk_compat_log_miss_cols(ctx, tab, j.d_rows, j.n_rows, d_vflag, j.vbeg, j.vend, j.d_mask, j.words, j.n_allele, 0,
                                     lut, j.table_cols, j.n_table_cols, j.d_L, j.d_miss8, j.ldm, j.d_flags);
      else
        rc = gk_compat_log_miss(ctx, tab, j.d_rows, j.n_rows, d_vflag, j.vbeg, j.vend, j.d_mask, j.words, j.n_allele, 0, lut,
                                j.d_L, j.d_miss8, j.ldm, j.d_flags);
    }
    if (rc == GK_OK && !summed) rc = gk_miss_colsum(ctx, j.d_miss8, j.ldm, nc, j.d_msum);
    if (rc == GK_OK && gk_fetch_queue(ctx, &flags[i], gk_ptr<void>(j.d_flags), sizeof(uint32_t)) != hipSuccess) rc = GK_ERR_HIP;
    if (rc) return rc;
    std::vector<int32_t> cols((size_t)nc);
    std::iota(cols.begin(), cols.end(), 0);
    if (gs[i]) gs[i]->abandon();
    gs[i].reset(new GeneSearch());
    rc = gs[i]->init(ctx, GkTable{j.d_L, j.n_rows, nullptr}, j.d_L, j.n_rows, j.n_rows, nc, j.d_miss8, j.ldm, j.d_msum,
                     cols.data(), nc, j.n_steps, j.top_n, argsort);
    if (rc == GK_OK) rc = gs[i]->colsum_enqueue();
    if (rc == GK_OK) rc = push(i, kTable);
    return rc;
  };
  std::vector<std::vector<int>> dependents((size_t)n_jobs);
  for (int i : live)
    if (jobs[i].table_of >= 0) dependents[(size_t)jobs[i].table_of].push_back(i);
  int rc = GK_OK;
  for (int i : live) {
    if (jobs[i].table_of >= 0) continue;
    rc = write_table(i, false);
    if (rc) return fail(rc);
  }

  auto advance = [&](int i, bool at_step_start) -> int {
    GeneSearch& g = *gs[i];
    for (;;) {
      if (at_step_start) {
        if (!g.more()) return GK_OK;
        const int r = g.step_begin();
        if (r) return r;
        if (g.bound_in_flight) return push(i, kBound);
      }
      if (!g.step_done) {
        const int r = g.exact_step();
        if (r) return r;
      }
      g.step_end();
      at_step_start = true;
    }
  };
  while (!queue.empty()) {
    const Item it = queue.front();
    queue.pop_front();
    clock.lap(false);
    rc = wait_mark(ctx, it.mark);
    clock.lap(true);
    if (rc) return fail(rc);
    const int at = it.stage == kOneSet ? batches[(size_t)it.gene]->deps[0] : it.gene;
    gk_gene_job& j = jobs[at];
    GeneSearch& g = *gs[at];
    switch (it.stage) {
      case kTable: {
        if (flags[it.gene] & 4u) {
          if (j.passes + j.patches >= 64) {
            gk_set_error("log10 value table did not settle");
            rc = GK_ERR_ASSERT;
            break;
          }
          rc = (j.passes + j.patches < 4 ? gk_lut_resolve_stored : gk_lut_resolve)(lut, log10_fn, nullptr, nullptr, nullptr);
          if (rc == GK_OK) rc = write_table(it.gene, (flags[it.gene] & 8u) == 0);
          break;
        }
        j.bound_ok = ((flags[it.gene] | sticky[it.gene]) & 1u) == 0 ? 1 : 0;
        if (!j.bound_ok) g.bound = false;
        g.colsum_collect();
        if (j.n_steps > 0) {
          rc = g.first_step();
          if (rc == GK_OK) rc = advance(it.gene, true);
        }
        const int nc = n_cols_of(it.gene);
        std::vector<int> one_set;
        for (int d : dependents[(size_t)it.gene]) {
          if (rc) break;
          gk_gene_job& jd = jobs[d];
          jd.bound_ok = j.bound_ok;
          bool single = jd.n_step_cols >= jd.n_steps && jd.n_steps >= 1;
          for (int q = 0; q < jd.n_steps && single; ++q) single = jd.step_cols_off[q + 1] - jd.step_cols_off[q] == 1;
          if (single) {
            gs[d].reset(new GeneSearch());
            gs[d]->S.reset(new gk_search());
            gs[d]->S->n_allele = nc;
            gs[d]->S->colsum = g.S->colsum;
            int32_t a0 = 0;
            rc = col_of(it.gene, jd.step_cols[jd.step_cols_off[0]], &a0);
            if (rc) break;
            Step s1;
            s1.n = 1;
            s1.value.push_back(g.S->colsum[(size_t)a0]);
            s1.sum_indv.push_back(g.S->colsum[(size_t)a0]);
            s1.ids.push_back(a0);
            s1.frac.push_back(1.0);
            gs[d]->S->steps.push_back(std::move(s1));
            if (jd.n_steps >= 2) one_set.push_back(d);
            continue;
          }
          gs[d].reset(new GeneSearch());
          std::vector<int32_t> every((size_t)nc);
          std::iota(every.begin(), every.end(), 0);
          rc = gs[d]->init(ctx, GkTable{j.d_L, j.n_rows, nullptr}, j.d_L, j.n_rows, j.n_rows, nc, j.d_miss8, j.ldm, j.d_msum,
                           every.data(), nc, jd.n_steps, jd.top_n, argsort);
          if (rc) break;
          if (!j.bound_ok) gs[d]->bound = false;
          gs[d]->S->colsum = g.S->colsum;
          if (jd.n_step_cols > 0) {
            gs[d]->step_cols.resize((size_t)jd.n_step_cols);
            for (int q = 0; q < jd.n_step_cols && rc == GK_OK; ++q) {
              std::vector<int32_t>& sc = gs[d]->step_cols[(size_t)q];
              sc.assign(jd.step_cols + jd.step_cols_off[q], jd.step_cols + jd.step_cols_off[q + 1]);
              for (int32_t& a : sc) { rc = col_of(it.gene, a, &a); if (rc) break; }
            }
            if (rc) break;
          }
          if (jd.n_steps > 0) {
            rc = gs[d]->first_step();
            if (rc == GK_OK) rc = advance(d, true);
          }
        }
        for (int k = 2; k <= 8 && rc == GK_OK; ++k) {
          std::unique_ptr<OneSetBatch> b(new OneSetBatch());
          b->k = k;
          for (int d : one_set) {
            if (jobs[d].n_steps < k) continue;
            for (int q = 0; q < k; ++q) {
              int32_t a = 0;
              const int r = col_of(it.gene, jobs[d].step_cols[jobs[d].step_cols_off[q]], &a);
              if (r) rc = r;
              b->ids.push_back(a);
            }
            b->deps.push_back(d);
          }
          if (rc || b->deps.empty()) break;
          rc = gk_shares_enqueue(ctx, GkTable{j.d_L, j.n_rows, nullptr}, j.n_rows, b->ids.data(), (int32_t)b->deps.size(), k, true,
                                 b->call);
          if (rc) break;
          gs[b->deps[0]]->S->note(b->call.leafwise ? 3 : 2, j.n_rows, (int64_t)b->deps.size(), k, gs[b->deps[0]]->S->distinct(b->ids.data(), b->ids.size()), 0, 0);
          batches.push_back(std::move(b));
          rc = push((int)batches.size() - 1, kOneSet);
        }
        break;
      }
      case kOneSet: {
        OneSetBatch& b = *batches[(size_t)it.gene];
        const int k = b.k;
        std::vector<double> value(b.deps.size()), frac(b.deps.size() * (size_t)k);
        gk_shares_collect(ctx, b.call, value.data(), frac.data());
        for (size_t x = 0; x < b.deps.size(); ++x) {
          gk_search& S = *gs[b.deps[x]]->S;
          Step st;
          st.n = k;
          st.bounded = 1;
          st.value.push_back(value[x]);
          for (int q = 0; q < k; ++q) {
            const int32_t a = b.ids[x * (size_t)k + q];
            st.ids.push_back(a);
            st.sum_indv.push_back(S.colsum[(size_t)a]);
            st.frac.push_back(frac[x * (size_t)k + q]);
          }
          S.steps.push_back(std::move(st));
        }
        break;
      }
      case kBound:
        rc = g.after_bound();
        if (rc == GK_OK) rc = g.sums_in_flight ? push(it.gene, kSums) : advance(it.gene, false);
        break;
      default:
        rc = g.after_sums();
        if (rc == GK_OK) rc = advance(it.gene, false);
        break;
    }
    if (rc) return fail(rc);
  }
  for (int i : live) {
    gs[i]->finish();
    const gk_gene_job& o = jobs[jobs[i].table_of >= 0 ? jobs[i].table_of : i];
    if (o.n_table_cols > 0) gs[i]->S->to_alleles(o.table_cols, o.n_table_cols, o.n_allele);
    out[i] = gs[i]->S.release();
  }
  clock.lap(false);
  return GK_OK;
}

}

extern "C" {

int gk_sample_search(gk_ctx* ctx, gk_ctx** more_ctx, int32_t n_more, gk_tab* tab, gk_dptr d_vflag, gk_lut* lut,
                     gk_gene_job* jobs, int32_t n_jobs, gk_argsort_fn argsort, gk_log10_fn log10_fn, gk_search** out) {
  gk_bind(ctx);
  GK_REQUIRE(ctx && tab && lut && jobs && argsort && log10_fn && out && n_jobs >= 0, "null pointer");
  GK_REQUIRE(n_more >= 0 && (n_more == 0 || more_ctx), "bad context list");
  std::vector<gk_ctx*> cx{ctx};
  for (int k = 0; k < n_more; ++k) {
    GK_REQUIRE(more_ctx[k] && more_ctx[k]->device == ctx->device, "contexts of one call share a device");
    cx.push_back(more_ctx[k]);
  }
  for (int i = 0; i < n_jobs; ++i) out[i] = nullptr;
  std::vector<int> live;
  bool any_special = false;
  for (int i = 0; i < n_jobs; ++i) {
    gk_gene_job& j = jobs[i];
    j.bound_ok = 0;
    j.passes = 0;
    j.indexed = 0;
    j.patches = 0;
    GK_REQUIRE(j.n_rows >= 0 && j.n_allele >= 0 && j.n_steps >= 0 && j.top_n >= 1, "bad gene job");
    GK_REQUIRE(j.table_of >= -1 && j.table_of < n_jobs && j.table_of != i, "bad table reference");
    GK_REQUIRE(j.n_step_cols >= 0 && (j.n_step_cols == 0 || (j.step_cols && j.step_cols_off)), "bad step columns");
    GK_REQUIRE(j.n_table_cols >= 0 && j.n_table_cols <= j.n_allele && (j.n_table_cols == 0 || j.table_cols), "bad table columns");
    GK_REQUIRE(j.n_table_cols == 0 || gk_compat_log_miss_cols, "column lists need the device build");
    for (int c = 0; c < j.n_table_cols; ++c)
      GK_REQUIRE(j.table_cols[c] >= 0 && j.table_cols[c] < j.n_allele && (c == 0 || j.table_cols[c] > j.table_cols[c - 1]),
                 "table columns must be allele ordinals, ascending and unique");
    if (j.table_of >= 0) {
      const gk_gene_job& o = jobs[j.table_of];
      GK_REQUIRE(o.table_of < 0, "a table reference must name a job that writes its own table");
      GK_REQUIRE(j.n_steps >= 1, "a search on another job's table needs steps");
      GK_REQUIRE(j.n_table_cols == 0, "a column list belongs to the job that writes the table");
      if (o.n_rows > 0 && o.n_allele > 0) { live.push_back(i); any_special = true; }
      continue;
    }
    if (j.n_steps == 0 || j.n_step_cols > 0 || j.n_table_cols > 0) any_special = true;
    if (j.n_rows > 0 && j.n_allele > 0) {
      GK_REQUIRE(j.d_rows && (j.d_L || j.d_lidx) && j.d_mask && j.words >= 1, "gene job without tables");
      GK_REQUIRE(!j.d_miss8 || (j.d_msum && j.d_flags && j.ldm >= j.n_rows && j.ldm % 64 == 0), "bad mismatch table");
      GK_REQUIRE(!j.d_lidx || j.d_miss8, "the index form comes with the mismatch table (same stride)");
      live.push_back(i);
    }
  }
  if (live.empty()) return GK_OK;
  bool float_tables = true;
  for (int i : live) if (jobs[i].table_of < 0) float_tables = float_tables && jobs[i].d_L && !jobs[i].d_lidx;
  bool flagged = true;
  for (int i : live) if (jobs[i].table_of < 0) flagged = flagged && jobs[i].d_miss8 && jobs[i].d_flags;
  if (n_more == 0 && float_tables && flagged)
    return sample_search_pipelined(ctx, tab, d_vflag, lut, jobs, n_jobs, live, argsort, log10_fn, out);
  GK_REQUIRE(!any_special, "table-only jobs, searches on another job's table, per-step columns and column lists need float64 tables "
                           "with mismatch tables on one stream (the pipelined form)");
  return sample_search_lockstep(ctx, cx, tab, d_vflag, lut, jobs, n_jobs, live, argsort, log10_fn, out);
}

int gk_search_steps(gk_search* s, int32_t* n_steps) {
  GK_REQUIRE(s && n_steps, "null pointer");
  *n_steps = (int32_t)s->steps.size();
  return GK_OK;
}

int gk_search_info(gk_search* s, int32_t step, int32_t* n, int64_t* rows, int32_t* bounded) {
  GK_REQUIRE(s && step >= 0 && step < (int32_t)s->steps.size() && n && rows && bounded, "bad search step");
  *n = s->steps[step].n;
  *rows = s->steps[step].rows();
  *bounded = s->steps[step].bounded;
  return GK_OK;
}

int gk_search_copy(gk_search* s, int32_t step, double* value, double* sum_indv, int32_t* ids, double* frac) {
  GK_REQUIRE(s && step >= 0 && step < (int32_t)s->steps.size(), "bad search step");
  const Step& st = s->steps[step];
  if (value) std::copy(st.value.begin(), st.value.end(), value);
  if (sum_indv) std::copy(st.sum_indv.begin(), st.sum_indv.end(), sum_indv);
  if (ids) std::copy(st.ids.begin(), st.ids.end(), ids);
  if (frac) std::copy(st.frac.begin(), st.frac.end(), frac);
  return GK_OK;
}

int gk_search_export(gk_search* const* s, int32_t n, int64_t* totals, int64_t* meta, double* value, double* sum_indv,
                     double* frac, int32_t* ids) {
  GK_REQUIRE(s && n >= 0 && totals, "null pointer");
  int64_t steps = 0, rows = 0, cells = 0;
  for (int q = 0; q < n; ++q) {
    GK_REQUIRE(s[q], "null search");
    for (const Step& st : s[q]->steps) { ++steps; rows += st.rows(); cells += st.rows() * st.n; }
  }
  totals[0] = steps; totals[1] = rows; totals[2] = cells;
  if (!meta) return GK_OK;
  GK_REQUIRE(value && sum_indv && frac && ids, "null pointer");
  int64_t* triple = meta + n;
  for (int q = 0; q < n; ++q) {
    meta[q] = (int64_t)s[q]->steps.size();
    for (const Step& st : s[q]->steps) {
      triple[0] = st.n; triple[1] = st.rows(); triple[2] = st.bounded;
      triple += 3;
      value = std::copy(st.value.begin(), st.value.end(), value);
      sum_indv = std::copy(st.sum_indv.begin(), st.sum_indv.end(), sum_indv);
      frac = std::copy(st.frac.begin(), st.frac.end(), frac);
      ids = std::copy(st.ids.begin(), st.ids.end(), ids);
    }
  }
  return GK_OK;
}

int gk_search_colsum(gk_search* s, double* out) {
  GK_REQUIRE(s && out, "null pointer");
  if (s->table_cols.empty()) {
    std::copy(s->colsum.begin(), s->colsum.end(), out);
    return GK_OK;
  }
  std::fill(out, out + s->n_full, std::nan(""));
  for (size_t c = 0; c < s->table_cols.size(); ++c) out[s->table_cols[c]] = s->colsum[c];
  return GK_OK;
}

int gk_search_log(gk_search* s, int64_t* out, int64_t capacity, int64_t* n_out) {
  GK_REQUIRE(s && n_out, "null pointer");
  *n_out = (int64_t)s->log.size();
  if (out) std::copy(s->log.begin(), s->log.begin() + std::min<int64_t>(capacity, *n_out), out);
  return GK_OK;
}

int gk_search_destroy(gk_search* s) {
  delete s;
  return GK_OK;
}

namespace {
struct SiteObs { int64_t pos, label; int64_t cnt; };

int sites_homozygous(std::vector<SiteObs>& obs, int32_t cn) {
  std::sort(obs.begin(), obs.end(), [](const SiteObs& a, const SiteObs& b) {
    return a.pos != b.pos ? a.pos < b.pos : a.label < b.label;
  });
  std::vector<int64_t> counts;
  for (size_t i = 0; i < obs.size();) {
    size_t j = i;
    counts.clear();
    int n_label = 0, n_positive = 0;
    while (j < obs.size() && obs[j].pos == obs[i].pos) {
      size_t q = j;
      int64_t c = 0;
      while (q < obs.size() && obs[q].pos == obs[i].pos && obs[q].label == obs[j].label) c += obs[q++].cnt;
      ++n_label;
      n_positive += (obs[j].label & 1) == 0;
      counts.push_back(c);
      j = q;
    }
    i = j;
    if (n_label <= 1 || n_positive == 0) continue;
    std::sort(counts.begin(), counts.end(), [](int64_t a, int64_t b) { return a > b; });
    int64_t total = 0;
    int kept = 0;
    for (int64_t c : counts)
      if (c > 3) { total += c; ++kept; }
    if (total < 20 || kept < 2) continue;
    const double second = (double)counts[1] / (double)total;
    if (!(second > 0.1)) continue;
    if (second > (1.0 / (double)(cn * 2))) return 0;
  }
  return 1;
}
}

int gk_site_verdict(const int64_t* pos, const int64_t* code, const uint8_t* negative, const int64_t* count, int64_t n,
                    int32_t cn, int32_t* homozygous) {
  GK_REQUIRE(homozygous && cn >= 1 && (n == 0 || (pos && code && negative && count)), "bad verdict arguments");
  *homozygous = 1;
  if (n == 0) return GK_OK;
  std::vector<SiteObs> obs((size_t)n);
  for (int64_t i = 0; i < n; ++i) obs[i] = SiteObs{pos[i], (code[i] << 1) | (negative[i] ? 1 : 0), count[i]};
// ... 48 lines not shown
```

kir_graph_amd/kir_typing.py:

```python
from __future__ import annotations

import contextlib
import ctypes as C
import json
import os
import sys
import threading
import time
from typing import Any

import numpy as np

from . import _lib
from ._lib import Device
from .call_bootstrap import MAX_BOOT, MAX_TOP, CallBootstrap, bootstrapCall, homoFactor
from .call_coverage import CallCoverage, coverCall
from .call_fit import MAX_EXTRA, CallFit, fitCall
from .engine import PreparedGene, PreparedSample, searchMode
from .hisat2 import SampleData, loadCompact, loadReadsAndVariantsData
from .typing_em import (EmBootstrap, Hisat2AlleleResult, bootstrapEM, callsByAbundance, candidateSetsDistinct,
                        hisat2TypingPerGene, summariseBootstrap)
from .typing_mulit_allele import (AlleleTyping, AlleleTypingExonFirst, ReadSet, StepList, isHetrozygous,
                                  sharedLogTable)
from .utils import NumpyEncoder, logger, testHook, traceOn
# ... 74 lines not shown
        self._rows = None
        if g is None:
            self._rows = (tab.dev.alloc(1, np.int32), 0)
            self.vbeg = self.n_span = 0
            self.mask, self.alleles, self.variants = None, [], []
            self.novel = lambda: []
            return
        t = idx.tables[g]
        self.vbeg, self.n_span = t.vbeg, t.vend - t.vbeg
        self.mask = tab.dindex.masks[g]
        self.alleles = t.alleles
        self.variants = idx.variants[t.vbeg:t.vend]
        self.novel = lambda: data.novelOfGene(gene)

    def _select(self):
        if self._rows is None:
            self._rows = self.tab.selectGene(self.g, self._multiple)
        return self._rows

    @property
    def rows(self):
        return self._select()[0]

    @property
    def n_rows(self) -> int:
        return self._select()[1]

    def prepared(self, prep: PreparedSample) -> PreparedGene:
        return prep.gene(self.g, self.vbeg, self.vbeg + self.n_span, self.tab.dev)

    def model(self, logs, prepared: PreparedGene | None = None, *, cls=AlleleTyping, variants=None, mask=None,
              alleles=None, **varying) -> AlleleTyping:
        if prepared is not None:
            reads = ReadSet(self.tab, prepared.rows, prepared.n_rows, prepared.vflag)
            varying["_prepared"] = prepared
        else:
            reads = ReadSet(self.tab, self.rows, self.n_rows)
        return cls(reads, self.variants if variants is None else variants, logs=logs, _vbeg=self.vbeg, _n_span=self.n_span,
                   _mask=self.mask if mask is None else mask, _alleles=self.alleles if alleles is None else alleles,
                   _novel=self.novel, **varying)

    def groupCache(self) -> dict:
        store = self.data.index.__dict__.setdefault("_exon_group_cache", {})
        return store.setdefault(self.gene, {})

    def exonFlags(self) -> np.ndarray:
        idx, tab = self.data.index, self.data.tab
        flags = np.full(tab.n_var_total, 3, dtype=np.uint8)
        flags[:idx.n_variant][idx.in_exon.astype(bool)] = 0
        return flags


class _OnLane(Typing):

    def __init__(self) -> None:
        super().__init__()
        self._local = threading.local()
        self.slot_base = 0
        self.tables_rewritten = 0
        self.tables_patched = 0

    def _context(self):
        tab = getattr(self._local, "tab", None)
        if tab is None:
            base = self._data.tab
            dev = base.dev.worker(self.slot_base)
            tab = self._local.tab = base.on(dev)
            self._local.logs = sharedLogTable(dev)
        return tab, self._local.logs


_SEARCH_SLOTS: dict = {}
_SEARCH_SLOTS_LOCK = threading.Lock()


def _searchSlot():
    n = int(os.environ.get("GK_SEARCH_SLOTS", "0") or 0)
    if n <= 0:
        return contextlib.nullcontext()
    with _SEARCH_SLOTS_LOCK:
        sem = _SEARCH_SLOTS.get(n)
        if sem is None:
            sem = _SEARCH_SLOTS[n] = threading.BoundedSemaphore(n)
    return sem


class TypingWithPosNegAllele(_OnLane):

    def __init__(self, filename_variant_json, top_n: int = 300, multiple: bool = False, exon_first: bool = False,
                 exon_only: bool = False, exon_candidate_threshold: float = .9, variant_correction: bool = False,
                 device: Device | None = None, call_bootstrap: int = 0, call_bootstrap_seed: int = 2022,
                 call_bootstrap_top: int = 32, call_fit: bool = False, call_fit_extra: int = 3,
                 call_coverage: bool = False, call_coverage_len: dict[str, int] | None = None):
        super().__init__()
        if call_coverage and not call_coverage_len:
            raise ValueError("call_coverage: needs call_coverage_len, the backbone length of every gene")
        self._call_coverage = (bool(call_coverage), dict(call_coverage_len or {}))
        self.call_coverage: dict[str, CallCoverage | None] = {}
        if not 0 <= int(call_fit_extra) <= MAX_EXTRA:
            raise ValueError(f"call_fit_extra: the extra alleles listed must lie in 0 .. {MAX_EXTRA}")
        self._call_fit = (bool(call_fit), int(call_fit_extra))
        self.call_fit: dict[str, CallFit] = {}
        if not 0 <= int(call_bootstrap) <= MAX_BOOT:
            raise ValueError(f"call_bootstrap: the number of replicates must lie in 0 .. {MAX_BOOT}")
        if not 1 <= int(call_bootstrap_top) <= MAX_TOP:
            raise ValueError(f"call_bootstrap_top: the candidate sets kept must lie in 1 .. {MAX_TOP}")
        self._call_boot = (int(call_bootstrap), int(call_bootstrap_seed), int(call_bootstrap_top))
        self.call_bootstrap: dict[str, CallBootstrap] = {}
        self._data = _sample(filename_variant_json, device)
        self._multiple = multiple
        self._top_n = top_n
        self._exon_first, self._exon_only = exon_first, exon_only
        self._exon_candidate_threshold = exon_candidate_threshold
        self._variant_correction = variant_correction

    def typing(self, gene_cn: dict[str, int], min_reads_num: int = 100) -> tuple[list[str], list[str]]:
        if self._wholeSample():
            return self._typingWholeSample(gene_cn, min_reads_num)
        if self._wholeSampleExonFirst():
            return self._typingWholeSampleExonFirst(gene_cn, min_reads_num)
        return super().typing(gene_cn, min_reads_num)

    def _wholeSampleExonFirst(self) -> bool:
        return (self._exon_first and not self._exon_only and os.environ.get("GK_INDEX_TABLE", "0") != "1"
                and searchMode() == "bound")

    def _typingWholeSampleExonFirst(self, gene_cn: dict[str, int], min_reads_num: int) -> tuple[list[str], list[str]]:
        full_tables = testHook("full_tables") is not None
        tab, logs = self._context()
        udev = tab.dev.urgent()
        prep_f = tab.prepared(udev, self._multiple)
        if prep_f is None:
            return super().typing(gene_cn, min_reads_num)
        prep_e = tab.prepared(udev, self._multiple, exon=True)
        top_n, threshold = self._top_n, self._exon_candidate_threshold
        todo = [(gene, int(cn)) for gene, cn in gene_cn.items() if cn]
        views = [_GeneView(self._data, gene, self._multiple, tab=tab) for gene, _ in todo]
        verd_e = self._zygosityVerdicts(tab, prep_e, [(v.g, cn) for v, (_, cn) in zip(views, todo)])

        plan: dict[int, dict] = {}
        jobs1 = []
        for k, ((gene, cn), view) in enumerate(zip(todo, views)):
            if view.g is None or not view.alleles:
                continue
            prepared_e, prepared_f = view.prepared(prep_e), view.prepared(prep_f)
            if prepared_e.n_rows == 0 or prepared_f.n_rows == 0:
                continue
            allele_group, grouped, group_names, exon_mask = AlleleTypingExonFirst.exonGroups(
                view.variants, view.n_span, view.groupCache(), tab.dev)
            force = False if isHetrozygous(gene) else None
            typ_e = view.model(logs, prepared_e, variants=grouped, mask=exon_mask, alleles=group_names, force_homo=force,
                               top_n=top_n, variant_correction=True, _defer_launch=True)
            job, homo = typ_e.geneJob(cn, verd_e.get(view.g) if cn > 1 else False)
            plan[k] = {"typ_e": typ_e, "homo_e": homo, "job1": len(jobs1), "groups": allele_group,
                       "full": prepared_f, "force": force}
            jobs1.append(job)
        self.tables_rewritten = self.tables_patched = 0
        self.exon_info: dict[str, dict] = {}
        if jobs1:
            with self._searchBatch(tab, logs, prep_e.vflag, jobs1) as (jobs, handles):
                for k, p in plan.items():
                    q = p["job1"]
                    p["typ_e"].adoptJob(jobs[q], C.c_void_p(handles[q]), todo[k][1], p["homo_e"])
        jobs2, keep_alive = [], []
        for k, p in plan.items():
            (gene, cn), view = todo[k], views[k]
            result = p["typ_e"].result[-1]
            result.setNameGroup(p["groups"])

            def full_model(table_cols=None):
                return view.model(logs, p["full"], force_homo=p["force"], top_n=top_n // 5, variant_correction=True,
                                  _defer_launch=True, _table_cols=table_cols)
            if not result.value.shape[0]:
                logger.warning("[Allele] Cannot typing with exon-only reads. Typing with exon+intron")
                p["full_model"] = full_model()
                p["fallback"] = True
                continue
            ranks = list(result.topRank(threshold=threshold))
            self.exon_info[gene] = {"exon_groups": len(p["groups"]), "exon_sets": int(result.value.shape[0]),
                                    "candidates": len(ranks)}
            if len(ranks) > 1024:
                p["per_gene"] = True
                continue
            allele_to_id = {a: i for i, a in enumerate(view.alleles)}
            cand_steps = [[np.ascontiguousarray([allele_to_id[a] for a in names], dtype=np.int32)
                           for names in result.allele_name_group[i]] for i in ranks]
            table_cols = np.unique(np.concatenate([c for steps in cand_steps for c in steps])).astype(np.int32)
            if full_tables or len(table_cols) == len(view.alleles):
                table_cols = None
            full = p["full_model"] = full_model(table_cols)
            self.exon_info[gene]["table_columns"] = len(view.alleles) if table_cols is None else len(table_cols)
            job, _ = full.geneJob(cn, False)
            job.n_steps = 0
            p["job2"] = len(jobs2)
            jobs2.append(job)
            p["cands"] = []
            for steps in cand_steps:
                cols = np.ascontiguousarray(np.concatenate(steps), dtype=np.int32)
                offs = np.ascontiguousarray(np.concatenate([[0], np.cumsum([len(x) for x in steps])]), dtype=np.int32)
                keep_alive += [cols, offs]
                cand = _lib.GeneJob(d_rows=job.d_rows, n_rows=job.n_rows, d_mask=job.d_mask, d_L=0, d_miss8=0, ldm=job.ldm,
                                    d_msum=0, d_flags=0, d_lidx=0, vbeg=job.vbeg, vend=job.vend, words=job.words,
                                    n_allele=job.n_allele, n_steps=len(steps), top_n=top_n // 5, bound_ok=0, passes=0,
                                    indexed=0, patches=0, table_of=p["job2"], n_step_cols=len(steps),
                                    step_cols=cols.ctypes.data, step_cols_off=offs.ctypes.data)
                p["cands"].append((len(jobs2), len(steps)))
                jobs2.append(cand)
        if jobs2:
            with self._searchBatch(tab, logs, prep_f.vflag, jobs2) as (jobs, handles):
                for k, p in plan.items():
                    if "job2" not in p:
                        continue
                    full = p["full_model"]
                    full.adoptTable(jobs[p["job2"]], C.c_void_p(handles[p["job2"]]))
                    steps = full.adoptSearches([handles[qc] for qc, _ in p["cands"]])
                    merged = steps.lastSteps().sortByScoreAndEveness()
                    merged.print()
                    results = StepList(p["typ_e"].result, steps, [merged])
                    p["results"], p["final"] = results, merged
        self._result = {}

        def entries():
            for k, (gene, cn) in enumerate(todo):
                p = plan.get(k)
                if p is None or p.get("per_gene"):
                    yield gene, *self.typingPerGene(gene, cn)
                    continue
                if p.get("fallback"):
                    p["full_model"]._model._launchLog()
                    final = p["full_model"].typing(cn)
                    self._result[gene] = p["typ_e"].result
                else:
                    self._result[gene], final = p["results"], p["final"]
                self._bootstrapCall(gene, cn, final)
                self._fitCall(gene, cn, final)
                self._coverCall(gene, cn, final)
                yield gene, _calls(gene, final), p["typ_e"].getReadsNum()
        calls = self._collect(entries(), min_reads_num)
        self._result = {gene: self._result[gene] for gene, _ in todo if gene in self._result}
        return calls

    def _wholeSample(self) -> bool:
        return not self._exon_first and not self._exon_only and self._variant_correction and searchMode() in ("bound", "exact")

    def _typingWholeSample(self, gene_cn: dict[str, int], min_reads_num: int) -> tuple[list[str], list[str]]:
        trace = traceOn("bench")
        t_in = time.perf_counter()
        tab, logs = self._context()
        prep = tab.prepared(tab.dev.urgent(), self._multiple)
        if prep is None:
            return super().typing(gene_cn, min_reads_num)
        t_prep = time.perf_counter()
        todo = [(gene, int(cn)) for gene, cn in gene_cn.items() if cn]
        entries = []
        views = [_GeneView(self._data, gene, self._multiple, tab=tab) for gene, _ in todo]
        verdicts = self._zygosityVerdicts(tab, prep, [(v.g, cn) for v, (_, cn) in zip(views, todo)])
        for (gene, cn), view in zip(todo, views):
            if view.g is None or not view.alleles:
                entries.append((gene, cn, None, None, False))
                continue
            prepared = view.prepared(prep)
            typ = view.model(logs, prepared, force_homo=False if isHetrozygous(gene) else None, top_n=self._top_n,
                             variant_correction=True, _defer_launch=True)
            if prepared.n_rows == 0:
                entries.append((gene, cn, typ, None, False))
                continue
            job, homo = typ.geneJob(cn, verdicts.get(view.g) if cn > 1 else False)
            entries.append((gene, cn, typ, job, homo))
        live = [e for e in entries if e[3] is not None]
        if live:
            if trace:
                print(f"[trace] pre {threading.get_native_id()} {t_in:.6f} {t_prep:.6f} {time.perf_counter():.6f}", file=sys.stderr, flush=True)
            self.tables_rewritten = self.tables_patched = 0
            with self._searchBatch(tab, logs, prep.vflag, [e[3] for e in live], more=(C.c_void_p * 1)()) as (jobs, handles):
                for k, (gene, cn, typ, _, homo) in enumerate(live):
                    typ.adoptJob(jobs[k], C.c_void_p(handles[k]), cn, homo)
        self._result = {}

        def calls():
            for gene, cn, typ, job, _ in entries:
                if typ is None:
                    self._result[gene] = []
                    yield gene, _noCall(gene, cn), 0
                    continue
                res = typ.result[-1] if job is not None else typ.typing(cn)
                self._result[gene] = typ.result
                self._bootstrapCall(gene, cn, res)
                self._fitCall(gene, cn, res)
                self._coverCall(gene, cn, res)
                yield gene, _calls(gene, res), typ.getReadsNum()
        return self._collect(calls(), min_reads_num)

    @contextlib.contextmanager
    def _searchBatch(self, tab, logs, vflag, job_list: list, more=None):
        jobs = (_lib.GeneJob * len(job_list))(*job_list)
        handles = (C.c_void_p * len(job_list))()
        try:
            with _searchSlot():
                _lib.check(_lib.lib().gk_sample_search(tab.dev.ctx, more, 0, tab.handle, vflag.ptr, logs.handle, jobs, len(jobs),
                                                       _lib.NUMPY_ARGSORT, _lib.NUMPY_LOG10, handles))
            self.tables_rewritten += sum(max(0, int(j.passes) - 1) for j in jobs)
            self.tables_patched += sum(int(j.patches) for j in jobs)
            yield jobs, handles
        finally:
            for h in handles:
                if h:
# ... 228 lines not shown
```

kir_graph_amd/roofmodel.py:

```python
from __future__ import annotations

HBM_PEAK_GBS = 8000.0
TILE = 32
N_SIMD = 256 * 4
NOMINAL_HZ = 2.4e9

ISSUE_CYCLES = {"v_mul_f64": 4.50, "v_add_f64": 4.26, "v_max_f64": 4.19, "v_bfe_i32": 4.43, "v_bfi_b32": 4.56,
                "v_sad_u8": 4.49}
GUIDE_CYCLES = {"v_mul_f64": 4.0, "v_add_f64": 4.0, "v_max_f64": 4.0, "v_bfe_i32": 2.0, "v_bfi_b32": 2.0, "v_sad_u8": 2.0}
SEQUENCE_CYCLES = {"compat_kernel": 5.81}
KERNEL_OPS = {
    "compat_kernel": ("v_bfe_i32", "v_bfi_b32", "v_bfi_b32", "v_mul_f64"),
    "minsum_sad": ("v_sad_u8",),
    "maxsum_chunks": ("v_max_f64", "v_add_f64"),
}


def laneOpsPeak(kernel: str, table: dict[str, float] = ISSUE_CYCLES) -> float:
    ops = KERNEL_OPS[kernel]
    return len(ops) * 64 * N_SIMD * NOMINAL_HZ / sum(table[o] for o in ops)


def symmetricOutputs(n: int) -> int:
    total = 0
    for t0 in range(0, n, TILE):
        rows = min(TILE, n - t0)
        total += rows * (n - t0)
    return total


def maxsumLaunch(n_rows: int, n_sets: int, c_prev: int, n_cols: int, n_prev_cols: int,
                 symmetric: bool = False) -> tuple[float, float]:
    by = 8.0 * n_rows * (n_cols + n_prev_cols) + 8.0 * n_sets * n_cols
    outputs = symmetricOutputs(n_cols) if symmetric else n_sets * n_cols
    return by, 2.0 * n_rows * outputs


def minsumLaunch(n_rows: int, n_sets: int, n_cols: int, n_prev_cols: int, symmetric: bool = False
                 ) -> tuple[float, float]:
    outputs = symmetricOutputs(n_cols) if symmetric else n_sets * n_cols
    return 1.0 * n_rows * (n_cols + n_prev_cols) + 4.0 * n_sets * n_cols, n_rows * outputs / 4.0


def compatLaunch(n_rows: int, n_allele: int, n_ids: float, out_bytes: int = 8) -> tuple[float, float]:
    return 4.0 * n_ids + 16.0 * n_rows + float(out_bytes + 1) * n_rows * n_allele, 4.0 * n_ids * n_allele


def tabLaunch(n_pairs: int, n_valid: int, n_ids: int, record_bytes: float | None = None) -> tuple[float, float]:
    read = 256.0 * n_pairs if record_bytes is None else float(record_bytes)
    return read + 4.0 * n_ids + 22.0 * n_valid, 0.0


def setsumLaunch(n_rows: int, n_sets: int, c: int, n_distinct: int) -> tuple[float, float]:
    return 8.0 * n_rows * n_distinct + 8.0 * n_sets * (c + 1), float(n_rows) * n_sets * (c + 1)


def emSetsLaunch(n_rows: int, n_ids: float, set_words: int) -> tuple[float, float]:
    return 24.0 * n_rows + 4.0 * n_ids + 4.0 * set_words, 0.0


def emVerifyLaunch(set_words: int) -> tuple[float, float]:
    return 4.0 * set_words, 0.0


def _priced(kernel: str, calls: list[tuple]) -> tuple[float, float, str, float]:
    by = ops = 0.0
    bound, peak = "hbm", 0.0
    for c in calls:
        if kernel == "maxsum_chunks":
            b, o = maxsumLaunch(*c[1:7])
            bound, peak = "valu", laneOpsPeak("maxsum_chunks")
        elif kernel == "colsum_chunks":
            b, o = 8.0 * c[1] * c[4] + 8.0 * c[4], 0.0
        elif kernel == "em_sets_groups":
            b, o = emSetsLaunch(*c[1:4])
        elif kernel == "em_sets_verify":
            b, o = emVerifyLaunch(c[3])
        elif kernel == "minsum_sad":
            b, o = minsumLaunch(*c[1:6])
            bound, peak = "valu", laneOpsPeak("minsum_sad")
        elif kernel == "compat_kernel":
            b, o = compatLaunch(*c[1:5])
            bound, peak = "valu", laneOpsPeak("compat_kernel")
        elif kernel == "compat_rows8":
            b, o = compatLaunch(*c[1:5])[0], 0.0
        elif kernel == "tab_count":
            b, o = tabLaunch(*c[1:5])
        elif kernel in ("fraction_chunks", "setsum_leaves"):
            b, o = setsumLaunch(*c[1:5])
        else:
            return 0.0, 0.0, "hbm", 0.0
        by += b
        ops += o
    return by, ops, bound, peak


def summarise(call_log: list[tuple], kernel: str, total_ms: float, launches: int) -> dict:
    calls = [c for c in call_log if c[0] == kernel]
    base = {"kernel": kernel, "bound": "hbm", "achieved": None, "peak": HBM_PEAK_GBS, "unit": "GB/s",
            "frac": None, "traffic": None, "launches": launches, "avg_launch_ms": total_ms / max(launches, 1)}
    if not calls or total_ms <= 0:
        return base
    by, ops, bound, peak = _priced(kernel, calls)
    if by <= 0:
        return base
    sec = total_ms / 1e3
    gbs = by / sec / 1e9
    hbm = {"achieved": gbs, "peak": HBM_PEAK_GBS, "unit": "GB/s", "frac": gbs / HBM_PEAK_GBS}
    out = dict(base)
    out["algorithmic_bytes_per_launch"] = by / max(launches, 1)
    if bound == "valu":
        tops = ops / sec / 1e12
        unit = {"maxsum_chunks": "Tops/s f64 (max+add)", "minsum_sad": "T lane-ops/s (v_sad_u8, 4 reads each)",
                "compat_kernel": "T lane-ops/s (4 VALU per id and allele)"}.get(kernel, "T lane-ops/s")
        guide = laneOpsPeak(kernel, GUIDE_CYCLES)
        out.update({"bound": "valu", "achieved": tops, "peak": peak / 1e12, "unit": unit, "frac": ops / sec / peak,
                    "peak_guide": guide / 1e12, "frac_guide": ops / sec / guide,
                    "issue_cycles": {o: ISSUE_CYCLES[o] for o in KERNEL_OPS[kernel]},
                    "algorithmic_ops_per_launch": ops / max(launches, 1), "hbm": hbm,
                    "note": "VALU-issue bound (ordered f64 products / a (max,+) or (min,+) contraction).  `peak` = the "
                            "kernel's own instruction mix issued back to back at the MEASURED cost of each instruction "
                            "(tools/valu_rate.hip at 8 waves per SIMD, profiles/r03_valu_rate.txt: cycles of a 2.4 GHz "
                            "clock per wave64 instruction and SIMD in `issue_cycles`); `peak_guide` / `frac_guide` price "
                            "the same mix at the guide's 2 cycles per 32-bit and 4 per float64 instruction.  The HBM "
                            "roof is shown beside it; symmetric launches are credited with the triangle of tiles they "
                            "compute"})
        if kernel in SEQUENCE_CYCLES:
            seq = 64 * N_SIMD * NOMINAL_HZ / SEQUENCE_CYCLES[kernel]
            out["peak_sequence"] = seq / 1e12
            out["frac_sequence"] = ops / sec / seq
            out["note"] += (".  `peak_sequence` / `frac_sequence`: the same instructions at the rate measured for them "
                            "as the sequence the kernel issues (eight independent chains per wave, 8 waves per SIMD)")
    else:
        out.update(hbm)
        out["bound"] = "hbm"
    return out


def dominant(prof: dict[str, tuple[int, float]], call_log: list[tuple]) -> dict:
    if not prof:
        return summarise([], "none", 0.0, 0)
    priced = {k: v for k, v in prof.items() if _priced(k, [c for c in call_log if c[0] == k])[0] > 0}
    top = max(prof.items(), key=lambda kv: kv[1][1])[0]
    name, (launches, total_ms) = max((priced or prof).items(), key=lambda kv: kv[1][1])
    out = summarise(call_log, name, total_ms, launches)
    total = sum(v[1] for v in prof.values())
    out["share_of_kernel_time"] = total_ms / total if total else None
    if top != name:
        out["largest_kernel_by_time"] = top
    others = {}
    for k, (n, ms) in prof.items():
        if k != name and ms > 0.02 * total:
            e = summarise(call_log, k, ms, n)
            if e.get("achieved") is not None:
                others[k] = {f: e[f] for f in ("bound", "achieved", "peak", "unit", "frac", "avg_launch_ms")}
    if others:
        out["other_kernels"] = others
    return out


def stepRoofline(call_log: list[tuple], steps: int, ms_per_step: float) -> dict:
    kernels = sorted({c[0] for c in call_log})
    total_bytes = hbm_floor = valu_floor = valu_floor_guide = 0.0
    per_kernel = {}
    for k in kernels:
        calls = [c for c in call_log if c[0] == k]
        by, ops, bound, peak = _priced(k, calls)
        if by <= 0:
            continue
        total_bytes += by
        hbm_floor += by / (HBM_PEAK_GBS * 1e9)
        if bound == "valu" and peak > 0:
            valu_floor += ops / peak
            valu_floor_guide += ops / laneOpsPeak(k, GUIDE_CYCLES)
        per_kernel[k] = {"bytes_per_step": by / max(steps, 1), "ops_per_step": ops / max(steps, 1), "bound": bound}
    steps = max(steps, 1)
    sec = ms_per_step / 1e3
    gbs = total_bytes / steps / sec / 1e9 if sec > 0 else None
    return {"algorithmic_bytes_per_step": total_bytes / steps, "achieved": gbs, "peak": HBM_PEAK_GBS, "unit": "GB/s",
            "frac": gbs / HBM_PEAK_GBS if gbs is not None else None,
            "hbm_floor_ms_per_step": 1e3 * hbm_floor / steps,
            "valu_floor_ms_per_step": 1e3 * valu_floor / steps,
            "valu_share_of_step": (1e3 * valu_floor / steps) / ms_per_step if ms_per_step > 0 else None,
            "valu_floor_ms_per_step_guide": 1e3 * valu_floor_guide / steps,
            "kernels": per_kernel,
            "note": "sum over all priced launches of one step (serial pass geometries) / the reported ms_per_step; the "
                    "step is VALU-issue bound, not HBM bound: valu_floor = the VALU-bound kernels' algorithmic "
                    "lane-operations at the measured issue peak of their instruction mix (…_guide: at the guide's price)"}
```

kir_graph_amd/typing_mulit_allele.py:

```python
from __future__ import annotations

from collections import defaultdict
from dataclasses import dataclass, field
from itertools import chain
from typing import Iterable, Optional

import threading

import numpy as np

from ._lib import Device, DeviceBuffer
from .engine import DeviceModel, LogTable, PreparedGene, Tabulation
from .index import buildMask
from .msa2hisat import Variant
from .utils import logger

SEARCH_STATS = {"bounded": 0, "redone_exactly": 0}
_default_logs: dict[int, LogTable] = {}
_default_logs_lock = threading.Lock()


def nativeSearch() -> bool:
    return True


def compatKernelOf(table_cols) -> str:
    import os
    if table_cols is None or not 0 < len(table_cols) <= 8:
        return "compat_kernel"
    hooks = os.environ.get("GK_TEST_HOOKS", "").split(",")
    return "compat_kernel" if "wide_compat" in hooks else "compat_rows8"


_GROUP_CACHE_LOCK = threading.Lock()


def sharedLogTable(dev: Device) -> LogTable:
    with _default_logs_lock:
        t = _default_logs.get(dev.ordinal)
        if t is None:
            t = _default_logs[dev.ordinal] = LogTable(dev, private_context=True)
    return t


@dataclass
class TypingResult:

    n: int
    value: np.ndarray
    value_sum_indv: np.ndarray
    allele_id: np.ndarray
    allele_name: list[list[str]]
    allele_prob: "np.ndarray | LazyAlleleProb"
    fraction: np.ndarray
    fraction_uniq: np.ndarray
    allele_name_group: list[list[list[str]]] = field(default_factory=list)

    def isFail(self) -> bool:
        return not len(self.value)

    def bestRank(self, filter_fraction: bool = True, filter_minor: bool = False) -> int:
        ids: Iterable[int] = range(len(self.fraction))
        if filter_fraction and len(self.fraction):
            floor = (1 / self.n) / 2
            ids = np.flatnonzero((np.asarray(self.fraction) >= floor).all(axis=1)).tolist()
        if filter_minor:
            ids = [i for i in ids
                   if np.abs(self.value_sum_indv[i]).min() / np.abs(self.value_sum_indv[i]).max() > 0.8]
        return (list(ids) or [0])[0]

    def selectBest(self, filter_fraction: bool = True, filter_minor: bool = False) -> list[str]:
        best = self.bestRank(filter_fraction, filter_minor)
        if not self.isFail():
            logger.debug(f"[Allele] Select best rank: {best}")
            assert len(self.allele_name[best]) == self.n
            return self.allele_name[best]
        logger.warning("[Allele] No candidates found. Return fail")
        return ["fail"] * self.n

    def print(self, num: int = 100, top_threshold: float = 0.9) -> None:
        if self.isFail():
            print("Fail Alleles:", ["fail"] * self.n)
            return
        if not logger.isEnabledFor(10):
            return
        lines = [f"Allele_num =  {self.n}"]
        for k, rank in enumerate(self.topRank(top_threshold)):
            if k > num:
                break
            lines.append(f"Rank {rank} probility {self.value[rank]} sum {self.value_sum_indv[rank].sum()}")
            for i in range(self.n):
                lines.append(f"  id {self.allele_id[rank][i]:3}   name {self.allele_name[rank][i]:20s}"
                             f"   fraction {self.fraction[rank][i]:.5f}   sum {self.value_sum_indv[rank][i]:8.3f}")
        logger.debug("[Allele] " + "\n".join(lines))

    def setNameGroup(self, allele_group_mapping: dict[str, list[str]]) -> None:
        self.allele_name_group = _GroupRows(self.allele_name, allele_group_mapping)

    def sortByScoreAndEveness(self, preserve_topn: int = -1) -> "TypingResult":
        if preserve_topn == -1:
            preserve_topn = self.value.shape[0]
        order = rankScore(self.value, self.value_sum_indv, self.fraction)[:preserve_topn]
        return TypingResult(
            n=self.n, value=self.value[order], value_sum_indv=self.value_sum_indv[order],
            allele_id=self.allele_id[order], allele_name=[self.allele_name[i] for i in order],
            allele_prob=takeColumns(self.allele_prob, order),
            fraction=self.fraction[order], fraction_uniq=self.fraction_uniq[order])

    def topRank(self, threshold: float = 0.9) -> Iterable[int]:
        assert not self.isFail()
        best = self.value[0]
        return [0] + [int(i) for i in np.nonzero(self.value[1:] * threshold >= best)[0] + 1]

    def selectAllPossible(self, threshold: float = 0.9) -> list[tuple[float, list[str]]]:
        if self.isFail():
            return []
        return [(self.value[r], self.allele_name[r]) for r in self.topRank(threshold)]


class _GroupRows:

    def __init__(self, names, mapping: dict[str, list[str]]):
        self._names, self._mapping = names, mapping

    def __len__(self) -> int:
        return len(self._names)

    def __getitem__(self, i):
        if isinstance(i, slice):
            return [self[k] for k in range(*i.indices(len(self)))]
        return [self._mapping[a] for a in self._names[i]]

    def __iter__(self):
        return (self[i] for i in range(len(self)))

    def __eq__(self, other) -> bool:
        return list(self) == list(other)


class SearchSteps:

    def __init__(self, typing, steps_of: np.ndarray, meta: np.ndarray, value, sum_indv, frac, ids):
        self._typing = typing
        self.steps_of = steps_of
        self.set_size, self.rows, self.bounded = meta[:, 0], meta[:, 1], meta[:, 2]
        self._value, self._sum_indv, self._frac, self._ids = value, sum_indv, frac, ids
        self.row0 = np.concatenate([[0], np.cumsum(self.rows)])
        self.cell0 = np.concatenate([[0], np.cumsum(self.rows * self.set_size)])
        self.first_step = np.concatenate([[0], np.cumsum(steps_of)])
        self.step_in_search = np.arange(len(self.rows)) - np.repeat(self.first_step[:-1], steps_of)
        self._made: dict[int, TypingResult] = {}

    def __len__(self) -> int:
        return len(self.rows)

    def __getitem__(self, j):
        if isinstance(j, slice):
            return [self[k] for k in range(*j.indices(len(self)))]
        if j < 0:
            j += len(self)
        got = self._made.get(j)
        if got is None:
            t = self._typing
            k, c = int(self.rows[j]), int(self.set_size[j])
            r0, c0 = int(self.row0[j]), int(self.cell0[j])
            ids = self._ids[c0:c0 + k * c].reshape(k, c)
            frac = self._frac[c0:c0 + k * c].reshape(k, c)
            got = self._made[j] = TypingResult(
                n=c, value=self._value[r0:r0 + k], value_sum_indv=self._sum_indv[c0:c0 + k * c].reshape(k, c), allele_id=ids,
                allele_name=LazyNames(ids, t.id_to_allele), allele_prob=LazyAlleleProb([(t._model, ids)]),
                fraction=frac if self.step_in_search[j] else np.ones(ids.shape), fraction_uniq=np.ones(ids.shape))
        return got

    def __iter__(self):
        return (self[j] for j in range(len(self)))

    def lastSteps(self) -> "TypingResult":
        last = self.first_step[1:] - 1
        c = int(self.set_size[last[0]])
        assert np.all(self.set_size[last] == c)
        k = self.rows[last]
        within = np.arange(int(k.sum())) - np.repeat(np.cumsum(k) - k, k)
        rows = np.repeat(self.row0[last], k) + within
        cells = (np.repeat(self.cell0[last], k) + within * c)[:, None] + np.arange(c)[None, :]
# ... 301 lines not shown

    @property
    def reads(self) -> list:
        if self._reads_cache is None:
            self._reads_cache = self._readset.hostReads(self._template)
        return self._reads_cache

    def getReadsNum(self) -> int:
        return self._model.n_rows

    @staticmethod
    def collectAlleleNames(variants: list[Variant]) -> set[str]:
        return set(chain.from_iterable(v.allele for v in variants))

    def mapAlleleIDs(self, list_ids: np.ndarray) -> list[list[str]]:
        return [[self.id_to_allele[int(i)] for i in ids] for ids in list_ids]

    def fork(self) -> "AlleleTyping":
        other = object.__new__(type(self))
        other.__dict__.update(self.__dict__)
        other.result = []
        return other

    def typing(self, cn: int) -> TypingResult:
        if cn < 1:
            raise ValueError(f"CN should be >= 1, got {cn}")
        homo = self._isHomozygous(cn) if self.force_homo is None else self.force_homo
        self.finish()
        self.result = []
        if homo:
            self.addCandidate()
            self.addHomoResultForCn(cn)
        else:
            if self._model.n_rows:
                self._searchNatively(cn)
            else:
                for _ in range(cn):
                    self.addCandidate()
        self.result[-1].print()
        return self.result[-1]

    def _searchNatively(self, cn: int) -> None:
        import ctypes as C
        from . import _lib
        from ._lib import check, lib
        m = self._model
        cols = np.arange(m.n_allele, dtype=np.int32)
        bound = m.boundOk
        colsum = None if self._colsum_all is None else np.ascontiguousarray(self._colsum_all, dtype=np.float64)
        h = C.c_void_p()
        check(lib().gk_search_run(m.dev.ctx, m.L.ptr, m.n_rows, m.n_rows, m.n_allele,
                                  m.miss8.ptr if bound else 0, m.ldm, m.msum.ptr if bound else 0,
                                  cols.ctypes.data, len(cols), cn, self.top_n, _lib.NUMPY_ARGSORT,
                                  None if colsum is None else colsum.ctypes.data, C.byref(h)))
        try:
            self._adoptSearch(h, cn)
        finally:
            lib().gk_search_destroy(h)

    def _adoptSearch(self, h, n_steps: int) -> None:
        import ctypes as C
        from ._lib import check, lib
        m = self._model
        if self._colsum_all is None:
            self._colsum_all = np.empty(m.n_allele, dtype=np.float64)
            check(lib().gk_search_colsum(h, self._colsum_all.ctypes.data))
        for step in range(n_steps):
            n, rows, bounded = C.c_int32(), C.c_int64(), C.c_int32()
            check(lib().gk_search_info(h, step, C.byref(n), C.byref(rows), C.byref(bounded)))
            k, c = int(rows.value), int(n.value)
            value = np.empty(k, dtype=np.float64)
            sum_indv, frac = np.empty((k, c), dtype=np.float64), np.empty((k, c), dtype=np.float64)
            ids32 = np.empty((k, c), dtype=np.int32)
            check(lib().gk_search_copy(h, step, value.ctypes.data, sum_indv.ctypes.data, ids32.ctypes.data,
                                       frac.ctypes.data))
            ids = ids32.astype(np.int64)
            if step:
                SEARCH_STATS["bounded" if bounded.value else "redone_exactly"] += 1
            self.result.append(TypingResult(
                n=c, value=value, value_sum_indv=sum_indv, allele_id=ids,
                allele_name=LazyNames(ids, self.id_to_allele), allele_prob=LazyAlleleProb([(m, ids)]),
                fraction=frac if step else np.ones(ids.shape), fraction_uniq=np.ones(ids.shape)))
        if m.dev.call_log is not None:
            self._logLaunches(h)

    def adoptSearches(self, handles: list, keep_log: bool = True) -> "SearchSteps":
        import ctypes as C
        from ._lib import check, lib
        m = self._model
        n = len(handles)
        arr = (C.c_void_p * max(n, 1))(*handles)
        totals = np.zeros(3, dtype=np.int64)
        check(lib().gk_search_export(arr, n, totals.ctypes.data, None, None, None, None, None))
        n_steps, n_rows, n_cells = (int(x) for x in totals)
        meta = np.zeros(n + 3 * n_steps, dtype=np.int64)
        value = np.empty(n_rows, dtype=np.float64)
        sum_indv, frac = np.empty(n_cells, dtype=np.float64), np.empty(n_cells, dtype=np.float64)
        ids = np.empty(n_cells, dtype=np.int32)
        check(lib().gk_search_export(arr, n, totals.ctypes.data, meta.ctypes.data, value.ctypes.data, sum_indv.ctypes.data,
                                     frac.ctypes.data, ids.ctypes.data))
        steps = SearchSteps(self, meta[:n], meta[n:].reshape(-1, 3), value, sum_indv, frac, ids.astype(np.int64))
        later = steps.step_in_search > 0
        SEARCH_STATS["bounded"] += int(np.count_nonzero(later & (steps.bounded != 0)))
        SEARCH_STATS["redone_exactly"] += int(np.count_nonzero(later & (steps.bounded == 0)))
        if keep_log and m.dev.call_log is not None:
            for h in handles:
                self._logLaunches(C.c_void_p(h))
        return steps

    def _logLaunches(self, h) -> None:
        import ctypes as C
        from ._lib import check, lib
        m = self._model
        n_log = C.c_int64()
        check(lib().gk_search_log(h, None, 0, C.byref(n_log)))
        raw = np.empty(n_log.value, dtype=np.int64)
        check(lib().gk_search_log(h, raw.ctypes.data, len(raw), C.byref(n_log)))
        for kind, a, b, c_, d, e, f in raw.reshape(-1, 7).tolist():
            if kind == 0:
                m.dev.call_log.append(("colsum_chunks" if b == 1 and c_ == 0 else "maxsum_chunks", a, b, c_, d, e, bool(f)))
            elif kind == 1:
                m.dev.call_log.append(("minsum_sad", a, b, c_, d, False))
            else:
                m.dev.call_log.append(("setsum_leaves" if kind == 3 else "fraction_chunks", a, b, c_, d))

    def geneJob(self, cn: int, verdict: bool | None = None):
        from ._lib import GeneJob
        if cn < 1:
            raise ValueError(f"CN should be >= 1, got {cn}")
        if self.force_homo is not None:
            homo = self.force_homo
        else:
            homo = self._isHomozygous(cn) if verdict is None else verdict
        m = self._model
        vbeg, vend, mask, words = m._geom
        cols = m._table_cols
        job = GeneJob(d_rows=m.rows.ptr, n_rows=m.n_rows, d_mask=mask.ptr, d_L=m._L.ptr if m._L else 0,
                      d_miss8=m.miss8.ptr if m.miss8 else 0, ldm=m.ldm, d_msum=m.msum.ptr if m.msum else 0,
                      d_flags=m._bound_flags.ptr if m._bound_flags else 0, d_lidx=m.lidx.ptr if m.lidx else 0,
                      vbeg=vbeg, vend=vend, words=words, n_allele=m.n_allele, n_steps=1 if homo else cn,
                      top_n=self.top_n, bound_ok=0, passes=0, indexed=0, patches=0, table_of=-1, n_step_cols=0,
                      step_cols=None, step_cols_off=None, table_cols=None if cols is None else cols.ctypes.data,
                      n_table_cols=0 if cols is None else len(cols))
        return job, homo

    def adoptJob(self, job, handle, cn: int, homo: bool) -> TypingResult:
        m = self._model
        m._bound_ok = bool(job.bound_ok)
        m._indexed = bool(job.indexed)
        m._known_at_launch = -1
        if m.dev.call_log is not None:
            per_row = m.tab.n_ids / max(m.tab.n_valid, 1)
            n_written = m.n_allele if m._table_cols is None else len(m._table_cols)
            for _ in range(max(1, int(job.passes))):
                m.dev.call_log.append((compatKernelOf(m._table_cols), m.n_rows, n_written, per_row * m.n_rows,
                                       2 if m._indexed else 8))
        self.result = []
        self._adoptSearch(handle, 1 if homo else cn)
        if homo:
            self.addHomoResultForCn(cn)
        self.result[-1].print()
        return self.result[-1]

    def adoptTable(self, job, handle) -> None:
        import ctypes as C
        from ._lib import check, lib
        m = self._model
        m._bound_ok = bool(job.bound_ok)
        m._indexed = False
        m._known_at_launch = -1
        n_written = m.n_allele if m._table_cols is None else len(m._table_cols)
        if m.dev.call_log is not None:
            per_row = m.tab.n_ids / max(m.tab.n_valid, 1)
            for _ in range(max(1, int(job.passes))):
                m.dev.call_log.append((compatKernelOf(m._table_cols), m.n_rows, n_written, per_row * m.n_rows, 8))
            self._logLaunches(handle)
        colsum = np.empty(m.n_allele, dtype=np.float64)
        check(lib().gk_search_colsum(handle, colsum.ctypes.data))
        self._colsum_all = colsum if m._table_cols is None else None
        self.result = []

    def addHomoResultForCn(self, cn: int) -> None:
        if cn > 1:
            self.result.append(self.createHomoResult(self.result[0], cn))

    @staticmethod
    def createHomoResult(cn1_result: TypingResult, cn: int) -> TypingResult:
        if cn <= 1:
            raise ValueError(f"CN should be > 1, got {cn}")
        if cn1_result.isFail():
            e = np.array([])
            return TypingResult(cn, e, e, e, [], e, e, e)
        m = len(cn1_result.value)
        return TypingResult(
            n=cn, value=cn1_result.value * cn,
            value_sum_indv=np.repeat(cn1_result.value_sum_indv, cn, axis=1),
            allele_id=np.repeat(cn1_result.allele_id, cn, axis=1),
            allele_name=[[row[0]] * cn for row in cn1_result.allele_name],
            allele_prob=cn1_result.allele_prob,
            fraction=np.ones((m, cn)) / cn, fraction_uniq=np.ones((m, cn)) / cn)

    @staticmethod
    def uniqueAllele(data: np.ndarray) -> np.ndarray:
        return firstOccurrence(np.asarray(data), int(np.max(data)) + 1 if np.size(data) else 1)

    def _colsums(self) -> np.ndarray:
        if self._colsum_all is None:
            self.finish()
            self._colsum_all = self._model.colsum(np.arange(self._model.n_allele))
        return self._colsum_all

    def addCandidate(self, candidate_allele: Optional[list[str]] = None) -> TypingResult:
        steps = self._candidateSteps(candidate_allele)
        try:
            request = next(steps)
            while True:
                request = steps.send(self._serve([request])[0])
        except StopIteration as done:
            return done.value

    def _serve(self, requests: list[tuple]) -> list[np.ndarray]:
        m = self._model
        kind = requests[0][0]
        assert all(r[0] == kind for r in requests)
        if kind == "fraction":
            ids = [np.asarray(r[1], dtype=np.int64) for r in requests]
            if len(ids) == 1:
                return [m.fraction(ids[0])]
            uniq, back = np.unique(np.concatenate(ids), axis=0, return_inverse=True)
            out = m.fraction(uniq)[back.ravel()]
            cuts = np.cumsum([len(x) for x in ids])[:-1]
            return np.split(out, cuts)
        prev = [np.asarray(r[1], dtype=np.int64) for r in requests]
        cols = [np.asarray(r[2], dtype=np.int64) for r in requests]
        if len(requests) == 1:
            return [m.maxsum(prev[0], cols[0])]
        union = np.unique(np.concatenate(cols))
        uniq, back = np.unique(np.concatenate(prev), axis=0, return_inverse=True)
        out = m.maxsum(uniq, union)
        back = back.ravel()
        blocks, row = [], 0
        for p_, c_ in zip(prev, cols):
            blocks.append(out[back[row:row + len(p_)]][:, np.searchsorted(union, c_)])
            row += len(p_)
        return blocks

    @staticmethod
    def runLockstep(searches: list[tuple["AlleleTyping", list]]) -> None:
        if not searches:
            return
        if len(searches) > 64:
            for i in range(0, len(searches), 64):
                AlleleTyping.runLockstep(searches[i:i + 64])
            return
        owner = searches[0][0]
        n_round = max(len(c) for _, c in searches)
        for k in range(n_round):
            active = [(model, model._candidateSteps(cands[k], allow_bound=False))
                      for model, cands in searches if k < len(cands)]
            pending = []
            for model, gen in active:
                try:
                    pending.append((gen, next(gen)))
                except StopIteration:
                    pass
            while pending:
                kinds = sorted({req[0] for _, req in pending})
                nxt = []
                for kind in kinds:
                    group = [(g, r) for g, r in pending if r[0] == kind]
                    answers = owner._serve([r for _, r in group])
                    for (g, _), ans in zip(group, answers):
                        try:
                            nxt.append((g, g.send(ans)))
                        except StopIteration:
                            pass
                pending = nxt

    def _boundedStep(self, prev: TypingResult, prev_ids: np.ndarray, cols: np.ndarray) -> Optional[TypingResult]:
        m, T = self._model, self.top_n
        first = firstOfSets(prev_ids, cols, m.n_allele)
        N = int(np.count_nonzero(first))
        if N == 0:
            return None
        sel = m.boundStep(prev_ids, cols, first, T, cap=4 * T + 4096)
        if sel is None:
            return None
        _, _, idx, _ = sel
        t_idx, a_idx = np.divmod(idx, len(cols))
        ids = np.concatenate([prev_ids[t_idx], cols[a_idx][:, None]], axis=1)
        value, frac = m.setsum(ids)
        n_top = min(max(T, N // 5), N)
        if N > T:
            v_cut = np.partition(value, len(value) - T)[len(value) - T]
            head = np.flatnonzero(value >= v_cut)
            if n_top > T:
                if len(head) > n_top:
                    return None
            elif len(head) != T:
                return None
        else:
            head = np.arange(len(value))
        ids, value, frac = ids[head], value[head], frac[head]
        sum_indv = self._colsums()[ids]
        key1, key2 = -value, -sum_indv.sum(axis=1)
        if len(head) > T:
            b = np.lexsort((key2, key1))[T - 1]
            contend = np.nonzero((key1 < key1[b]) | ((key1 == key1[b]) & (key2 <= key2[b])))[0]
        else:
            contend = np.arange(len(head))
        fc = frac[contend]
        uneven = np.abs(fc - fc.mean(axis=1, keepdims=True)).sum(axis=1)
        k1, k2 = key1[contend], key2[contend]
        sub = np.lexsort((uneven, k2, k1))
        look = sub[:T + 1]
        same = (k1[look][1:] == k1[look][:-1]) & (k2[look][1:] == k2[look][:-1]) & \
               (uneven[look][1:] == uneven[look][:-1])
        if same.any():
            return None
        sub = sub[:T]
        order = contend[sub]
        kept = ids[order]
        res = TypingResult(
            n=prev.n + 1, value=value[order], value_sum_indv=sum_indv[order], allele_id=kept,
            allele_name=LazyNames(kept, self.id_to_allele), allele_prob=LazyAlleleProb([(m, kept)]),
            fraction=fc[sub], fraction_uniq=np.ones(kept.shape))
        return res

# ... 342 lines not shown
```

Baseline: 516.5 million.

## Deduplicate identical reads into classes before computing the per-allele likelihood table

Adds a GPU pass that hashes each read's filtered variant-id set, verifies the hash matches, and assigns each read a class with one representative row. When a gene has many rows and columns and the classes number at most an eighth of the rows, the compat likelihood kernels run only on the representatives. An expand kernel then scatters the results back into the full L, mismatch and column-sum tables. This trades a hashing pass, an extra expand pass, a host wait on the class count and temporary allocations for far less per-allele work when reads repeat.

```diff
diff --git a/include/graphkir_hip.h b/include/graphkir_hip.h
--- a/include/graphkir_hip.h
+++ b/include/graphkir_hip.h
@@ -199,6 +199,10 @@
                               int32_t vbeg, int32_t vend, gk_dptr d_mask, int32_t words, int32_t n_allele,
                               int32_t keep_empty, gk_lut* lut, const int32_t* table_cols, int32_t n_table_cols,
                               gk_dptr d_log, gk_dptr d_miss8, int64_t ldm, gk_dptr d_flags, gk_dptr d_msum);
+int gk_row_classes(gk_ctx* ctx, gk_tab* tab, gk_dptr d_rows, int64_t n_rows, gk_dptr d_vflag, gk_dptr d_cls, gk_dptr d_rep,
+                   gk_dptr d_count, int32_t* n_classes_out);
+int gk_expand_classes(gk_ctx* ctx, gk_dptr d_Lc, int64_t n_classes, gk_dptr d_cls, int64_t n_rows, int32_t n_cols, gk_dptr d_L,
+                      gk_dptr d_miss8, int64_t ldm, gk_dptr d_msum);
 int gk_compat_patch(gk_ctx* ctx, gk_lut* lut, gk_dptr d_log, int64_t n_rows, int32_t n_allele, gk_dptr d_miss8,
                     int64_t ldm, gk_dptr d_flags);
 int gk_compat_index(gk_ctx* ctx, gk_tab* tab, gk_dptr d_rows, int64_t n_rows, gk_dptr d_vflag, int32_t vbeg,
@@ -237,6 +241,9 @@
   const int32_t* step_cols_off;
   const int32_t* table_cols;
   int32_t n_table_cols;
+  int32_t n_classes;
+  int32_t classified;
+  int32_t classify;
 } gk_gene_job;
 int gk_sample_search(gk_ctx* ctx, gk_ctx** more_ctx, int32_t n_more, gk_tab* tab, gk_dptr d_vflag, gk_lut* lut,
                      gk_gene_job* jobs, int32_t n_jobs, gk_argsort_fn argsort, gk_log10_fn log10_fn, gk_search** out);
diff --git a/kir_graph_amd/_lib.py b/kir_graph_amd/_lib.py
--- a/kir_graph_amd/_lib.py
+++ b/kir_graph_amd/_lib.py
@@ -50,7 +50,7 @@
         ("n_steps", C.c_int32), ("top_n", C.c_int32), ("bound_ok", C.c_int32), ("passes", C.c_int32),
         ("indexed", C.c_int32), ("patches", C.c_int32),
         ("table_of", C.c_int32), ("n_step_cols", C.c_int32), ("step_cols", C.c_void_p), ("step_cols_off", C.c_void_p),
-        ("table_cols", C.c_void_p), ("n_table_cols", C.c_int32),
+        ("table_cols", C.c_void_p), ("n_table_cols", C.c_int32), ("n_classes", C.c_int32), ("classified", C.c_int32), ("classify", C.c_int32),
     ]
 
 
@@ -203,6 +203,10 @@
                                      C.c_uint64, C.c_int32, C.c_int32, C.c_int32, C.c_void_p, C.c_uint64, C.c_uint64,
                                      C.c_int64, C.c_uint64]),
     "gk_miss_colsum": (C.c_int, [C.c_void_p, C.c_uint64, C.c_int64, C.c_int32, C.c_uint64]),
+    "gk_row_classes": (C.c_int, [C.c_void_p, C.c_void_p, C.c_uint64, C.c_int64, C.c_uint64, C.c_uint64, C.c_uint64, C.c_uint64,
+                                 C.POINTER(C.c_int32)]),
+    "gk_expand_classes": (C.c_int, [C.c_void_p, C.c_uint64, C.c_int64, C.c_uint64, C.c_int64, C.c_int32, C.c_uint64, C.c_uint64,
+                                    C.c_int64, C.c_uint64]),
     "gk_compat_index": (C.c_int, [C.c_void_p, C.c_void_p, C.c_uint64, C.c_int64, C.c_uint64, C.c_int32, C.c_int32,
                                   C.c_uint64, C.c_int32, C.c_int32, C.c_int32, C.c_void_p, C.c_uint64, C.c_uint64,
                                   C.c_int64, C.c_uint64]),
diff --git a/kir_graph_amd/build.py b/kir_graph_amd/build.py
--- a/kir_graph_amd/build.py
+++ b/kir_graph_amd/build.py
@@ -10,7 +10,7 @@
 SOURCES = ["gk_runtime.hip", "gk_scan.hip", "gk_tabulate.hip", "gk_typing.hip", "gk_lut.hip",
            "gk_search.hip", "gk_bound.hip", "gk_em.hip", "gk_cn.hip", "gk_depth.hip", "gk_sampack.cpp", "gk_bamread.cpp", "gk_textout.cpp",
            "gk_comm.cpp", "gk_hostsearch.cpp", "gk_novel.hip", "gk_boot.hip", "gk_callboot.hip", "gk_compat_narrow.hip",
-           "gk_callfit.hip", "gk_callcov.hip"]
+           "gk_callfit.hip", "gk_callcov.hip", "gk_rowclass.hip"]
 
 
 def hipcc() -> str:
@@ -32,6 +32,10 @@
     "compat_kernel": ["gk_typing.hip", "gk_lut.h", "gk_common.h"],
     "patch_pending": ["gk_typing.hip", "gk_lut.h", "gk_common.h"],
     "compat_rows8": ["gk_compat_narrow.hip", "gk_lut.h", "gk_common.h"],
+    "row_hash_claim": ["gk_rowclass.hip", "gk_common.h"],
+    "row_verify": ["gk_rowclass.hip", "gk_common.h"],
+    "row_number": ["gk_rowclass.hip", "gk_common.h"],
+    "expand_classes": ["gk_rowclass.hip", "gk_common.h"],
     "count_ids_genes": ["gk_typing.hip", "gk_common.h"],
     "flag_nonempty": ["gk_typing.hip", "gk_common.h"],
     "flag_pairs": ["gk_typing.hip", "gk_common.h"],
diff --git a/kir_graph_amd/csrc/gk_hostsearch.cpp b/kir_graph_amd/csrc/gk_hostsearch.cpp
--- a/kir_graph_amd/csrc/gk_hostsearch.cpp
+++ b/kir_graph_amd/csrc/gk_hostsearch.cpp
@@ -200,6 +200,10 @@
                                                     int32_t keep_empty, gk_lut* lut, const int32_t* table_cols,
                                                     int32_t n_table_cols, gk_dptr d_log, gk_dptr d_miss8, int64_t ldm,
                                                     gk_dptr d_flags, gk_dptr d_msum);
+__attribute__((weak)) int gk_row_classes(gk_ctx* ctx, gk_tab* tab, gk_dptr d_rows, int64_t n_rows, gk_dptr d_vflag, gk_dptr d_cls,
+                                         gk_dptr d_rep, gk_dptr d_count, int32_t* n_classes_out);
+__attribute__((weak)) int gk_expand_classes(gk_ctx* ctx, gk_dptr d_Lc, int64_t n_classes, gk_dptr d_cls, int64_t n_rows,
+                                            int32_t n_cols, gk_dptr d_L, gk_dptr d_miss8, int64_t ldm, gk_dptr d_msum);
 int gk_miss_colsum(gk_ctx* ctx, gk_dptr d_miss8, int64_t ldm, int32_t n_cols, gk_dptr d_msum);
 int gk_compat_patch(gk_ctx* ctx, gk_lut* lut, gk_dptr d_log, int64_t n_rows, int32_t n_allele, gk_dptr d_miss8, int64_t ldm,
                     gk_dptr d_flags);
@@ -776,6 +780,10 @@
   return GK_OK;
 }
 
+constexpr int64_t kClassMinRows = 131072;
+constexpr int kClassMinCols = 9;
+constexpr int64_t kClassShareNum = 1, kClassShareDen = 8;
+
 int sample_search_pipelined(gk_ctx* ctx, gk_tab* tab, gk_dptr d_vflag, gk_lut* lut, gk_gene_job* jobs, int32_t n_jobs,
                             const std::vector<int>& live, gk_argsort_fn argsort, gk_log10_fn log10_fn, gk_search** out) {
   SearchClock clock("pipelined", (int)live.size());
@@ -786,10 +794,47 @@
   std::deque<Item> queue;
   struct OneSetBatch { GkSumCall call; std::vector<int> deps; int k = 0; std::vector<int32_t> ids; };
   std::vector<std::unique_ptr<OneSetBatch>> batches;
+  struct RowClasses {
+    void *cls = nullptr, *rep = nullptr, *count = nullptr;
+    uint32_t n = 0;
+    uint64_t mark = 0;
+    bool queued = false;
+    hipEvent_t ev[4] = {nullptr, nullptr, nullptr, nullptr};
+  };
+  std::vector<RowClasses> classes((size_t)n_jobs);
+  static const bool plain_tables = gk_test_hook("plain_tables"), class_tables = gk_test_hook("class_tables");
+  static const bool trace_classes = gk_trace("classes");
+  auto stamp = [&](int i, int k) {
+    if (!trace_classes) return;
+    hipEvent_t& e = classes[(size_t)i].ev[k];
+    if (!e && hipEventCreate(&e) != hipSuccess) { e = nullptr; return; }
+    (void)hipEventRecord(e, ctx->stream);
+  };
+  auto drop_classes = [&]() {
+    for (RowClasses& c : classes) {
+      gk_pool_free(ctx, c.cls); gk_pool_free(ctx, c.rep); gk_pool_free(ctx, c.count);
+      for (hipEvent_t e : c.ev) if (e) (void)hipEventDestroy(e);
+      c = RowClasses();
+    }
+  };
+  auto report_classes = [&]() {
+    if (!trace_classes) return;
+    for (int i = 0; i < n_jobs; ++i) {
+      const RowClasses& c = classes[(size_t)i];
+      if (!c.ev[2] || !c.ev[3]) continue;
+      float ms_class = 0.f, ms_table = 0.f;
+      if (c.ev[0] && c.ev[1]) (void)hipEventElapsedTime(&ms_class, c.ev[0], c.ev[1]);
+      (void)hipEventElapsedTime(&ms_table, c.ev[2], c.ev[3]);
+      fprintf(stderr, "[row classes] job %d: %lld rows, %d columns, %u classes, form %s, classify %.3f ms, table %.3f ms\n", i,
+              (long long)jobs[i].n_rows, jobs[i].n_table_cols > 0 ? jobs[i].n_table_cols : jobs[i].n_allele, c.n,
+              jobs[i].n_classes > 0 ? "classes" : "plain", ms_class, ms_table);
+    }
+  };
   auto fail = [&](int code) {
     gk_fetch_cancel(ctx);
     for (auto& g : gs) if (g) g->abandon();
     for (auto& b : batches) if (b) gk_release(ctx, b->call.temps);
+    drop_classes();
     return code;
   };
   auto push = [&](int gene, int stage) {
@@ -826,16 +871,41 @@
       j.passes++;
       sticky[i] = 0;
       static const bool wide_compat = gk_test_hook("wide_compat");
+      const RowClasses& rc_of = classes[(size_t)i];
+      const bool by_class = rc_of.queued && rc_of.n >= 1 && (int64_t)rc_of.n <= j.n_rows &&
+                            (class_tables || (int64_t)rc_of.n * kClassShareDen <= j.n_rows * kClassShareNum);
+      j.n_classes = by_class ? (int32_t)rc_of.n : 0;
+      const int64_t t_rows = by_class ? (int64_t)rc_of.n : j.n_rows;
+      const int64_t t_ldm = by_class ? (t_rows + 63) / 64 * 64 : j.ldm;
+      const gk_dptr t_list = by_class ? gk_addr(rc_of.rep) : j.d_rows;
+      void *Lc = nullptr, *mc = nullptr, *sums = nullptr;
+      gk_dptr t_L = j.d_L, t_miss8 = j.d_miss8, t_msum = j.d_msum;
+      if (by_class) {
+        if (gk_pool_malloc(ctx, &Lc, (size_t)nc * (size_t)t_rows * sizeof(double)) != hipSuccess ||
+            gk_pool_malloc(ctx, &mc, (size_t)nc * (size_t)t_ldm) != hipSuccess ||
+            gk_pool_malloc(ctx, &sums, (size_t)nc * sizeof(uint32_t)) != hipSuccess) {
+          gk_pool_free(ctx, Lc); gk_pool_free(ctx, mc); gk_pool_free(ctx, sums);
+          gk_set_error("out of device memory for the class table of a gene");
+          return GK_ERR_HIP;
+        }
+        t_L = gk_addr(Lc); t_miss8 = gk_addr(mc); t_msum = gk_addr(sums);
+      }
       if (j.n_table_cols > 0 && j.n_table_cols <= 8 && gk_compat_log_miss_narrow && !wide_compat) {
-        rc = gk_compat_log_miss_narrow(ctx, tab, j.d_rows, j.n_rows, d_vflag, j.vbeg, j.vend, j.d_mask, j.words, j.n_allele, 0,
-                                       lut, j.table_cols, j.n_table_cols, j.d_L, j.d_miss8, j.ldm, j.d_flags, j.d_msum);
+        rc = gk_compat_log_miss_narrow(ctx, tab, t_list, t_rows, d_vflag, j.vbeg, j.vend, j.d_mask, j.words, j.n_allele, 0,
+                                       lut, j.table_cols, j.n_table_cols, t_L, t_miss8, t_ldm, j.d_flags, t_msum);
         summed = true;
       } else if (j.n_table_cols > 0)
-        rc = gk_compat_log_miss_cols(ctx, tab, j.d_rows, j.n_rows, d_vflag, j.vbeg, j.vend, j.d_mask, j.words, j.n_allele, 0,
-                                     lut, j.table_cols, j.n_table_cols, j.d_L, j.d_miss8, j.ldm, j.d_flags);
+        rc = gk_compat_log_miss_cols(ctx, tab, t_list, t_rows, d_vflag, j.vbeg, j.vend, j.d_mask, j.words, j.n_allele, 0,
+                                     lut, j.table_cols, j.n_table_cols, t_L, t_miss8, t_ldm, j.d_flags);
       else
-        rc = gk_compat_log_miss(ctx, tab, j.d_rows, j.n_rows, d_vflag, j.vbeg, j.vend, j.d_mask, j.words, j.n_allele, 0, lut,
-                                j.d_L, j.d_miss8, j.ldm, j.d_flags);
+        rc = gk_compat_log_miss(ctx, tab, t_list, t_rows, d_vflag, j.vbeg, j.vend, j.d_mask, j.words, j.n_allele, 0, lut,
+                                t_L, t_miss8, t_ldm, j.d_flags);
+      if (by_class) {
+        if (rc == GK_OK)
+          rc = gk_expand_classes(ctx, t_L, t_rows, gk_addr(rc_of.cls), j.n_rows, nc, j.d_L, j.d_miss8, j.ldm, j.d_msum);
+        summed = true;
+        gk_pool_free(ctx, Lc); gk_pool_free(ctx, mc); gk_pool_free(ctx, sums);
+      }
     }
     if (rc == GK_OK && !summed) rc = gk_miss_colsum(ctx, j.d_miss8, j.ldm, nc, j.d_msum);
     if (rc == GK_OK && gk_fetch_queue(ctx, &flags[i], gk_ptr<void>(j.d_flags), sizeof(uint32_t)) != hipSuccess) rc = GK_ERR_HIP;
@@ -855,8 +925,36 @@
     if (jobs[i].table_of >= 0) dependents[(size_t)jobs[i].table_of].push_back(i);
   int rc = GK_OK;
   for (int i : live) {
+    gk_gene_job& j = jobs[i];
+    if (j.table_of >= 0 || plain_tables || !gk_row_classes || !gk_expand_classes) continue;
+    if (!class_tables && (!j.classify || j.n_rows < kClassMinRows || n_cols_of(i) < kClassMinCols)) continue;
+    RowClasses& c = classes[(size_t)i];
+    if (gk_pool_malloc(ctx, &c.cls, (size_t)j.n_rows * sizeof(int32_t)) != hipSuccess ||
+        gk_pool_malloc(ctx, &c.rep, (size_t)j.n_rows * sizeof(int32_t)) != hipSuccess ||
+        gk_pool_malloc(ctx, &c.count, sizeof(uint32_t)) != hipSuccess) {
+      gk_set_error("out of device memory for the row classes of a gene");
+      return fail(GK_ERR_HIP);
+    }
+    stamp(i, 0);
+    rc = gk_row_classes(ctx, tab, j.d_rows, j.n_rows, d_vflag, gk_addr(c.cls), gk_addr(c.rep), gk_addr(c.count), nullptr);
+    stamp(i, 1);
+    if (rc == GK_OK && gk_fetch_queue(ctx, &c.n, c.count, sizeof(uint32_t)) != hipSuccess) rc = GK_ERR_HIP;
+    if (rc == GK_OK) rc = set_mark(ctx, &c.mark);
+    if (rc) return fail(rc);
+    c.queued = true;
+    j.classified = 1;
+  }
+  for (int i : live) {
     if (jobs[i].table_of >= 0) continue;
+    if (classes[(size_t)i].queued) {
+      clock.lap(false);
+      rc = wait_mark(ctx, classes[(size_t)i].mark);
+      clock.lap(true);
+      if (rc) return fail(rc);
+    }
+    stamp(i, 2);
     rc = write_table(i, false);
+    stamp(i, 3);
     if (rc) return fail(rc);
   }
 
@@ -1015,6 +1113,8 @@
     if (o.n_table_cols > 0) gs[i]->S->to_alleles(o.table_cols, o.n_table_cols, o.n_allele);
     out[i] = gs[i]->S.release();
   }
+  report_classes();
+  drop_classes();
   clock.lap(false);
   return GK_OK;
 }
@@ -1042,6 +1142,8 @@
     j.passes = 0;
     j.indexed = 0;
     j.patches = 0;
+    j.n_classes = 0;
+    j.classified = 0;
     GK_REQUIRE(j.n_rows >= 0 && j.n_allele >= 0 && j.n_steps >= 0 && j.top_n >= 1, "bad gene job");
     GK_REQUIRE(j.table_of >= -1 && j.table_of < n_jobs && j.table_of != i, "bad table reference");
     GK_REQUIRE(j.n_step_cols >= 0 && (j.n_step_cols == 0 || (j.step_cols && j.step_cols_off)), "bad step columns");
diff --git a/kir_graph_amd/csrc/gk_rowclass.hip b/kir_graph_amd/csrc/gk_rowclass.hip
--- /dev/null
+++ b/kir_graph_amd/csrc/gk_rowclass.hip
@@ -0,0 +1,324 @@
+#include <algorithm>
+
+#include "gk_common.h"
+
+namespace {
+
+constexpr int kThreads = 256;
+constexpr int kGroup = 16;
+constexpr int kGroups = kThreads / kGroup;
+constexpr int kWindow = 128;
+constexpr uint32_t kNoRow = 0xFFFFFFFFu;
+constexpr uint32_t kSignBit = 0x80000000u;
+
+__device__ inline uint64_t mix64(uint64_t x) {
+  x ^= x >> 30; x *= 0xBF58476D1CE4E5B9ull;
+  x ^= x >> 27; x *= 0x94D049BB133111EBull;
+  return x ^ (x >> 31);
+}
+
+__device__ inline uint32_t group_ballot(bool p) {
+  return (uint32_t)(__ballot(p) >> ((threadIdx.x & 63) & ~(kGroup - 1))) & 0xFFFFu;
+}
+
+constexpr int kDeep = 4;
+constexpr uint32_t kRound = kGroup * kDeep;
+struct Round { uint32_t pair[kDeep]; bool keep[kDeep]; };
+__device__ inline Round round_at(const uint32_t* __restrict__ ids, const uint8_t* __restrict__ vflag, uint32_t k0, uint32_t mid,
+                                 uint32_t e, int lane) {
+  Round r;
+  uint32_t v[kDeep];
+  uint8_t f[kDeep];
+#pragma unroll
+  for (int j = 0; j < kDeep; ++j) {
+    const uint32_t k = k0 + (uint32_t)lane + kGroup * j;
+    v[j] = ids[k < e ? k : e - 1u];
+  }
+#pragma unroll
+  for (int j = 0; j < kDeep; ++j) f[j] = vflag[v[j]];
+#pragma unroll
+  for (int j = 0; j < kDeep; ++j) {
+    const uint32_t k = k0 + (uint32_t)lane + kGroup * j;
+    const bool positive = k < mid;
+    r.pair[j] = v[j] | (positive ? kSignBit : 0u);
+    r.keep[j] = k < e && !(f[j] & (positive ? 1 : 2));
+  }
+  return r;
+}
+
+__global__ __launch_bounds__(kThreads) void row_hash_claim(const int32_t* __restrict__ rows, int64_t n_rows,
+                                                           const uint32_t* __restrict__ off, const uint32_t* __restrict__ ids,
+                                                           const uint8_t* __restrict__ vflag, unsigned long long* keys,
+                                                           uint32_t* minrow, uint64_t slot_mask, uint64_t hash_mask,
+                                                           uint32_t* __restrict__ slot_of) {
+  const int lane = threadIdx.x & (kGroup - 1);
+  const int64_t i = (int64_t)blockIdx.x * kGroups + threadIdx.x / kGroup;
+  if (i >= n_rows) return;
+  const int64_t row = rows[i];
+  const uint32_t b = off[4 * row], mid = off[4 * row + 2], e = off[4 * row + 4];
+  uint64_t h = 0;
+  uint32_t n = 0;
+  for (uint32_t k0 = b; k0 < e; k0 += kRound) {
+    const Round r = round_at(ids, vflag, k0, mid, e, lane);
+#pragma unroll
+    for (int j = 0; j < kDeep; ++j) {
+      h += r.keep[j] ? mix64((uint64_t)r.pair[j] + 0x9E3779B97F4A7C15ull) : 0ull;
+      n += r.keep[j] ? 1u : 0u;
+    }
+  }
+#pragma unroll
+  for (int d = kGroup / 2; d > 0; d >>= 1) {
+    h += __shfl_xor(h, d, kGroup);
+    n += __shfl_xor(n, d, kGroup);
+  }
+  if (lane != 0) return;
+  h = mix64(h + n) & hash_mask;
+  if (++h == 0ull) h = 1ull;
+  uint64_t s = mix64(h) & slot_mask;
+  for (;;) {
+    unsigned long long seen = __atomic_load_n(&keys[s], __ATOMIC_RELAXED);
+    if (seen == 0ull) seen = atomicCAS(&keys[s], 0ull, (unsigned long long)h);
+    if (seen == 0ull || seen == h) break;
+    s = (s + 1) & slot_mask;
+  }
+  if (__atomic_load_n(&minrow[s], __ATOMIC_RELAXED) > (uint32_t)i) atomicMin(&minrow[s], (uint32_t)i);
+  slot_of[i] = (uint32_t)s;
+}
+
+__global__ __launch_bounds__(kThreads) void row_verify(const int32_t* __restrict__ rows, int64_t n_rows,
+                                                       const uint32_t* __restrict__ off, const uint32_t* __restrict__ ids,
+                                                       const uint8_t* __restrict__ vflag, const uint32_t* __restrict__ minrow,
+                                                       uint32_t* slot_rep, uint32_t* __restrict__ self) {
+  __shared__ uint32_t window[kGroups][kWindow];
+  const int lane = threadIdx.x & (kGroup - 1);
+  const int g = threadIdx.x / kGroup;
+  const int64_t i = (int64_t)blockIdx.x * kGroups + g;
+  if (i >= n_rows) return;
+  const uint32_t p = minrow[slot_rep[i]];
+  bool same = true;
+  if ((int64_t)p != i) {
+    const int64_t row_i = rows[i], row_p = rows[p];
+    const uint32_t bi = off[4 * row_i], mi = off[4 * row_i + 2], ei = off[4 * row_i + 4];
+    const uint32_t bp = off[4 * row_p], mp = off[4 * row_p + 2], ep = off[4 * row_p + 4];
+    const uint32_t below = (1u << lane) - 1u;
+    uint32_t kp = bp, cp = 0, ki = bi, ci = 0;
+    uint32_t* const buf = window[g];
+    auto ranks = [&](const Round& r, uint32_t before, uint32_t (&t)[kDeep]) {
+      uint32_t c = before;
+#pragma unroll
+      for (int j = 0; j < kDeep; ++j) {
+        const uint32_t bal = group_ballot(r.keep[j]);
+        t[j] = c + (uint32_t)__builtin_popcount(bal & below);
+        c += (uint32_t)__builtin_popcount(bal);
+      }
+      return c - before;
+    };
+    Round ri;
+    bool have_ri = ki < ei;
+    if (have_ri) ri = round_at(ids, vflag, ki, mi, ei, lane);
+    for (;;) {
+      const uint32_t t0 = cp;
+      while (kp < ep) {
+        const Round r = round_at(ids, vflag, kp, mp, ep, lane);
+        uint32_t t[kDeep];
+        const uint32_t n = ranks(r, cp, t);
+        if (cp + n - t0 > (uint32_t)kWindow) break;
+#pragma unroll
+        for (int j = 0; j < kDeep; ++j)
+          if (r.keep[j]) buf[t[j] - t0] = r.pair[j];
+        cp += n;
+        kp += kRound;
+      }
+      const uint32_t t1 = cp;
+      const bool last = kp >= ep;
+      __builtin_amdgcn_wave_barrier();
+      while (ki < ei) {
+        if (!have_ri) ri = round_at(ids, vflag, ki, mi, ei, lane);
+        have_ri = false;
+        uint32_t t[kDeep];
+        const uint32_t n = ranks(ri, ci, t);
+        bool bad = false;
+#pragma unroll
+        for (int j = 0; j < kDeep; ++j) {
+          const bool inside = ri.keep[j] && t[j] >= t0 && t[j] < t1;
+          const uint32_t want = buf[inside ? t[j] - t0 : 0u];
+          bad = bad || (inside && want != ri.pair[j]) || (ri.keep[j] && t[j] >= t1 && last);
+        }
+        if (group_ballot(bad)) { same = false; break; }
+        if (ci + n > t1) { have_ri = true; break; }
+        ci += n;
+        ki += kRound;
+      }
+      __builtin_amdgcn_wave_barrier();
+      if (!same) break;
+      if (last) { same = ki >= ei && ci == t1; break; }
+    }
+  }
+  if (lane == 0) {
+    slot_rep[i] = same ? p : (uint32_t)i;
+    self[i] = (same && (int64_t)p != i) ? 0u : 1u;
+  }
+}
+
+__global__ __launch_bounds__(kThreads) void row_number(const int32_t* __restrict__ rows, int64_t n_rows,
+                                                       const uint32_t* __restrict__ rep_of, const uint32_t* __restrict__ pos,
+                                                       int32_t* __restrict__ cls, int32_t* __restrict__ d_rep) {
+  const int64_t i = (int64_t)blockIdx.x * kThreads + threadIdx.x;
+  if (i >= n_rows) return;
+  const uint32_t r = rep_of[i];
+  const uint32_t c = pos[r];
+  cls[i] = (int32_t)c;
+  if ((int64_t)r == i) d_rep[c] = rows[i];
+}
+
+constexpr int kExpandRows = 4 * kThreads;
+constexpr int kExpandCols = 32;
+
+__global__ __launch_bounds__(kThreads) void expand_classes(const double* __restrict__ Lc, int64_t n_classes,
+                                                           const int32_t* __restrict__ cls, int64_t n_rows, int n_cols,
+                                                           double* __restrict__ L, uint8_t* __restrict__ miss8, int64_t ldm,
+                                                           uint32_t* msum) {
+  __shared__ uint32_t col_sum[kExpandCols];
+  const int tid = threadIdx.x;
+  if (tid < kExpandCols) col_sum[tid] = 0;
+  __syncthreads();
+  const int64_t r0 = (int64_t)blockIdx.x * kExpandRows + 4 * tid;
+  const int c0 = blockIdx.y * kExpandCols, c1 = min(c0 + kExpandCols, n_cols);
+  const int n_r = (int)max((int64_t)0, min((int64_t)4, n_rows - r0));
+  int32_t k[4];
+#pragma unroll
+  for (int j = 0; j < 4; ++j) k[j] = cls[r0 + j < n_rows ? r0 + j : n_rows - 1];
+  const bool mine = r0 < ldm;
+  {
+    for (int c = c0; c < c1; ++c) {
+      const double* const src = Lc + (int64_t)c * n_classes;
+      double v[4];
+      uint32_t m[4];
+#pragma unroll
+      for (int j = 0; j < 4; ++j) v[j] = src[k[j]];
+#pragma unroll
+      for (int j = 0; j < 4; ++j) {
+        const double t = __builtin_fma(v[j], -1.0 / 3.0, 0.25);
+        m[j] = t < 100.0 ? (uint32_t)(int)t : 255u;
+      }
+      uint32_t packed = 0, sum = 0;
+#pragma unroll
+      for (int j = 0; j < 4; ++j)
+        if (j < n_r) { packed |= m[j] << (8 * j); sum += m[j]; }
+      double* const dst = L + (int64_t)c * n_rows + r0;
+      if (!mine) {
+        sum = 0;
+      } else if (n_r == 4) {
+        if ((((int64_t)c * n_rows) & 1) == 0) {
+          reinterpret_cast<double2*>(dst)[0] = make_double2(v[0], v[1]);
+          reinterpret_cast<double2*>(dst)[1] = make_double2(v[2], v[3]);
+        } else {
+#pragma unroll
+          for (int j = 0; j < 4; ++j) dst[j] = v[j];
+        }
+      } else {
+#pragma unroll
+        for (int j = 0; j < 4; ++j)
+          if (j < n_r) dst[j] = v[j];
+      }
+      if (mine) *reinterpret_cast<uint32_t*>(miss8 + (int64_t)c * ldm + r0) = packed;
+#pragma unroll
+      for (int d = 32; d > 0; d >>= 1) sum += __shfl_xor(sum, d, 64);
+      if ((tid & 63) == 0 && sum) atomicAdd(&col_sum[c - c0], sum);
+    }
+  }
+  __syncthreads();
+  if (tid < c1 - c0 && col_sum[tid]) atomicAdd(&msum[c0 + tid], col_sum[tid]);
+}
+
+}
+
+extern "C" {
+
+int gk_row_classes(gk_ctx* ctx, gk_tab* tab, gk_dptr d_rows, int64_t n_rows, gk_dptr d_vflag, gk_dptr d_cls, gk_dptr d_rep,
+                   gk_dptr d_count, int32_t* n_classes_out) {
+  gk_bind(ctx);
+  GK_REQUIRE(ctx && tab && d_count, "null pointer");
+  GK_REQUIRE(n_rows >= 0 && n_rows < ((int64_t)1 << 31), "bad row count");
+  uint32_t* const count = gk_ptr<uint32_t>(d_count);
+  if (n_rows == 0) {
+    GK_HIP(hipMemsetAsync(count, 0, sizeof(uint32_t), ctx->stream));
+    if (n_classes_out) {
+      GK_HIP(hipStreamSynchronize(ctx->stream));
+      *n_classes_out = 0;
+    }
+    return GK_OK;
+  }
+  GK_REQUIRE(d_rows && d_vflag && d_cls && d_rep, "null pointer");
+  static const bool weak_hash = gk_test_hook("weak_row_hash");
+  uint64_t slots = 64;
+  while (slots < 2 * (uint64_t)n_rows) slots <<= 1;
+  unsigned long long* keys = nullptr;
+  uint32_t *minrow = nullptr, *slot_rep = nullptr, *pos = nullptr;
+  auto release = [&]() {
+    gk_pool_free(ctx, keys); gk_pool_free(ctx, minrow); gk_pool_free(ctx, slot_rep); gk_pool_free(ctx, pos);
+  };
+  if (gk_pool_malloc(ctx, (void**)&keys, slots * sizeof(unsigned long long)) != hipSuccess ||
+      gk_pool_malloc(ctx, (void**)&minrow, slots * sizeof(uint32_t)) != hipSuccess ||
+      gk_pool_malloc(ctx, (void**)&slot_rep, (size_t)n_rows * sizeof(uint32_t)) != hipSuccess ||
+      gk_pool_malloc(ctx, (void**)&pos, (size_t)(n_rows + 1) * sizeof(uint32_t)) != hipSuccess) {
+    release();
+    gk_set_error("out of device memory for the row classes");
+    return GK_ERR_HIP;
+  }
+  int rc = GK_OK;
+  do {
+    if (hipMemsetAsync(keys, 0, slots * sizeof(unsigned long long), ctx->stream) != hipSuccess ||
+        hipMemsetAsync(minrow, 0xFF, slots * sizeof(uint32_t), ctx->stream) != hipSuccess) {
+      gk_set_error("row classes: clearing the hash table failed: %s", hipGetErrorString(hipGetLastError()));
+      rc = GK_ERR_HIP;
+      break;
+    }
+    const dim3 by_group((unsigned)((n_rows + kGroups - 1) / kGroups)), by_thread((unsigned)((n_rows + kThreads - 1) / kThreads));
+    GK_PROF(ctx, "row_hash_claim",
+            GK_KERNEL(row_hash_claim, by_group, dim3(kThreads), 0, ctx->stream, gk_ptr<int32_t>(d_rows), n_rows, tab->d_off,
+                      tab->d_ids, gk_ptr<uint8_t>(d_vflag), keys, minrow, slots - 1, weak_hash ? 15ull : ~0ull, slot_rep));
+    GK_PROF(ctx, "row_verify",
+            GK_KERNEL(row_verify, by_group, dim3(kThreads), 0, ctx->stream, gk_ptr<int32_t>(d_rows), n_rows, tab->d_off,
+                      tab->d_ids, gk_ptr<uint8_t>(d_vflag), minrow, slot_rep, pos));
+    rc = gk_scan_u32(ctx, pos, n_rows, count);
+    if (rc) break;
+    GK_PROF(ctx, "row_number",
+            GK_KERNEL(row_number, by_thread, dim3(kThreads), 0, ctx->stream, gk_ptr<int32_t>(d_rows), n_rows, slot_rep, pos,
+                      gk_ptr<int32_t>(d_cls), gk_ptr<int32_t>(d_rep)));
+    if (hipGetLastError() != hipSuccess) {
+      gk_set_error("row classes: a launch failed");
+      rc = GK_ERR_HIP;
+    }
+  } while (false);
+  release();
+  if (rc) return rc;
+  if (n_classes_out) {
+    uint32_t d = 0;
+    if (gk_fetch(ctx, &d, count, sizeof(uint32_t)) != hipSuccess) {
+      gk_set_error("row classes: fetching the class count failed");
+      return GK_ERR_HIP;
+    }
+    *n_classes_out = (int32_t)d;
+  }
+  return GK_OK;
+}
+
+int gk_expand_classes(gk_ctx* ctx, gk_dptr d_Lc, int64_t n_classes, gk_dptr d_cls, int64_t n_rows, int32_t n_cols, gk_dptr d_L,
+                      gk_dptr d_miss8, int64_t ldm, gk_dptr d_msum) {
+  gk_bind(ctx);
+  GK_REQUIRE(ctx, "null pointer");
+  if (n_rows == 0 || n_cols == 0) return GK_OK;
+  GK_REQUIRE(d_Lc && d_cls && d_L && d_miss8 && d_msum, "null pointer");
+  GK_REQUIRE(n_rows > 0 && n_cols > 0 && n_classes >= 1 && n_classes <= n_rows, "bad class table");
+  GK_REQUIRE(ldm >= n_rows && ldm % 64 == 0, "mismatch table stride must be a multiple of 64 rows");
+  GK_HIP(hipMemsetAsync(gk_ptr<uint32_t>(d_msum), 0, (size_t)n_cols * sizeof(uint32_t), ctx->stream));
+  const dim3 grid((unsigned)((ldm + kExpandRows - 1) / kExpandRows), (unsigned)((n_cols + kExpandCols - 1) / kExpandCols));
+  GK_PROF(ctx, "expand_classes",
+          GK_KERNEL(expand_classes, grid, dim3(kThreads), 0, ctx->stream, gk_ptr<double>(d_Lc), n_classes, gk_ptr<int32_t>(d_cls), n_rows, n_cols, gk_ptr<double>(d_L), gk_ptr<uint8_t>(d_miss8), ldm,
+                    gk_ptr<uint32_t>(d_msum)));
+  GK_HIP(hipGetLastError());
+  return GK_OK;
+}
+
+}
diff --git a/kir_graph_amd/kir_typing.py b/kir_graph_amd/kir_typing.py
--- a/kir_graph_amd/kir_typing.py
+++ b/kir_graph_amd/kir_typing.py
@@ -250,6 +250,7 @@
             typ_e = view.model(logs, prepared_e, variants=grouped, mask=exon_mask, alleles=group_names, force_homo=force,
                                top_n=top_n, variant_correction=True, _defer_launch=True)
             job, homo = typ_e.geneJob(cn, verd_e.get(view.g) if cn > 1 else False)
+            job.classify = 1
             plan[k] = {"typ_e": typ_e, "homo_e": homo, "job1": len(jobs1), "groups": allele_group,
                        "full": prepared_f, "force": force}
             jobs1.append(job)
diff --git a/kir_graph_amd/roofmodel.py b/kir_graph_amd/roofmodel.py
--- a/kir_graph_amd/roofmodel.py
+++ b/kir_graph_amd/roofmodel.py
@@ -44,6 +44,14 @@
 
 def compatLaunch(n_rows: int, n_allele: int, n_ids: float, out_bytes: int = 8) -> tuple[float, float]:
     return 4.0 * n_ids + 16.0 * n_rows + float(out_bytes + 1) * n_rows * n_allele, 4.0 * n_ids * n_allele
+
+
+def rowClassesLaunch(n_rows: int, n_ids: float) -> tuple[float, float]:
+    return 2.0 * (4.0 * n_ids + 16.0 * n_rows), 0.0
+
+
+def expandClassesLaunch(n_rows: int, n_classes: int, n_cols: int) -> tuple[float, float]:
+    return 9.0 * n_rows * n_cols + 9.0 * n_classes * n_cols, 0.0
 
 
 def tabLaunch(n_pairs: int, n_valid: int, n_ids: int, record_bytes: float | None = None) -> tuple[float, float]:
@@ -84,6 +92,10 @@
             bound, peak = "valu", laneOpsPeak("compat_kernel")
         elif kernel == "compat_rows8":
             b, o = compatLaunch(*c[1:5])[0], 0.0
+        elif kernel == "row_classes":
+            b, o = rowClassesLaunch(*c[1:3])
+        elif kernel == "expand_classes":
+            b, o = expandClassesLaunch(*c[1:4])
         elif kernel == "tab_count":
             b, o = tabLaunch(*c[1:5])
         elif kernel in ("fraction_chunks", "setsum_leaves"):
diff --git a/kir_graph_amd/typing_mulit_allele.py b/kir_graph_amd/typing_mulit_allele.py
--- a/kir_graph_amd/typing_mulit_allele.py
+++ b/kir_graph_amd/typing_mulit_allele.py
@@ -30,6 +30,17 @@
         return "compat_kernel"
     hooks = os.environ.get("GK_TEST_HOOKS", "").split(",")
     return "compat_kernel" if "wide_compat" in hooks else "compat_rows8"
+
+
+def logTableLaunches(call_log: list, job, table_cols, n_rows: int, n_written: int, per_row: float, out_bytes: int = 8) -> None:
+    classes = int(job.n_classes)
+    if int(job.classified):
+        call_log.append(("row_classes", n_rows, per_row * n_rows))
+    for _ in range(max(1, int(job.passes))):
+        taken = classes if classes > 0 else n_rows
+        call_log.append((compatKernelOf(table_cols), taken, n_written, per_row * taken, out_bytes))
+        if classes > 0:
+            call_log.append(("expand_classes", n_rows, classes, n_written))
 
 
 _GROUP_CACHE_LOCK = threading.Lock()
@@ -637,9 +648,7 @@
         if m.dev.call_log is not None:
             per_row = m.tab.n_ids / max(m.tab.n_valid, 1)
             n_written = m.n_allele if m._table_cols is None else len(m._table_cols)
-            for _ in range(max(1, int(job.passes))):
-                m.dev.call_log.append((compatKernelOf(m._table_cols), m.n_rows, n_written, per_row * m.n_rows,
-                                       2 if m._indexed else 8))
+            logTableLaunches(m.dev.call_log, job, m._table_cols, m.n_rows, n_written, per_row, 2 if m._indexed else 8)
         self.result = []
         self._adoptSearch(handle, 1 if homo else cn)
         if homo:
@@ -657,8 +666,7 @@
         n_written = m.n_allele if m._table_cols is None else len(m._table_cols)
         if m.dev.call_log is not None:
             per_row = m.tab.n_ids / max(m.tab.n_valid, 1)
-            for _ in range(max(1, int(job.passes))):
-                m.dev.call_log.append((compatKernelOf(m._table_cols), m.n_rows, n_written, per_row * m.n_rows, 8))
+            logTableLaunches(m.dev.call_log, job, m._table_cols, m.n_rows, n_written, per_row)
             self._logLaunches(handle)
         colsum = np.empty(m.n_allele, dtype=np.float64)
         check(lib().gk_search_colsum(handle, colsum.ctypes.data))
```

Result: slower. 475.0 million (-8.0%).
